# VisionDepth/VisionDepth3D

Hardware: AMD Instinct MI355X
Metric: stereo-pairs/sec end-to-end (depth+warp+fill+mux) (higher is better)
Workload: dtype f32; 1 GPU; 4k-dav2b-dibr; frame=3840x2160, format=Half-SBS, depth_model=depth-anything-v2-base, depth_net_dtype=float32 (the reference's precision), pixel_overlap=True, pixel_streams=2, clip_frames_all_ranks=32, params=render_cli.py defaults + dof_strength 2.0, dense DOF order (parity mode)

## Files before the change

include/vd3d.h:

```cpp
#ifndef VD3D_H
#define VD3D_H

#include <stddef.h>
#include <stdint.h>

#ifdef __cplusplus
extern "C" {
#endif

#define VD3D_ABI_VERSION 6

typedef enum vd3d_status {
  VD3D_OK = 0,
  VD3D_E_INVALID = -1,
  VD3D_E_HIP = -2,
  VD3D_E_NOMEM = -3,
  VD3D_E_UNSUPPORTED = -4
} vd3d_status;

typedef enum vd3d_format {
  VD3D_FMT_HALF_SBS = 0,
  VD3D_FMT_FULL_SBS = 1,
  VD3D_FMT_VR = 2,
  VD3D_FMT_ANAGLYPH = 3,
// ... 93 lines not shown
void vd3d_render_params_default(vd3d_render_params* p);

#define VD3D_STREAM_PRIVATE ((void*)(intptr_t)-1)
int vd3d_ctx_create(int device, void* stream, vd3d_ctx** out);
int vd3d_ctx_destroy(vd3d_ctx* ctx);
int vd3d_sync(vd3d_ctx* ctx);
void* vd3d_ctx_stream(vd3d_ctx* ctx);
int vd3d_ctx_set_stream(vd3d_ctx* ctx, void* stream);
void* vd3d_ctx_pixel_stream(vd3d_ctx* ctx);
void* vd3d_ctx_pixel_stream_k(vd3d_ctx* ctx, int k);

int vd3d_state_reset(vd3d_ctx* ctx);
int vd3d_state_new_clip(vd3d_ctx* ctx);
int vd3d_state_export(vd3d_ctx* ctx, vd3d_state* host_out);
int vd3d_state_import(vd3d_ctx* ctx, const vd3d_state* host_in);
int vd3d_state_planes(vd3d_ctx* ctx, float** tdf_prev, float** norm_prev, int* eye_h, int* eye_w);
int vd3d_last_scalars(vd3d_ctx* ctx, vd3d_frame_scalars* host_out);

int vd3d_pixel_shift(vd3d_ctx* ctx, const float* rgb_chw, const float* depth, int in_h, int in_w,
                     int W, int H, const vd3d_shift_params* p,
                     uint8_t* left_bgr, uint8_t* right_bgr, float* shift_or_null);

int vd3d_render_frame(vd3d_ctx* ctx, const uint8_t* frame_bgr, const void* depth, int depth_fmt,
                      const vd3d_render_params* p, uint8_t* out_bgr);

int vd3d_render_frame_blank(vd3d_ctx* ctx, const uint8_t* frame_bgr, const void* depth, int depth_fmt,
                            const vd3d_render_params* p, uint8_t* out_bgr);

int vd3d_shard_begin(vd3d_ctx* ctx, const vd3d_render_params* p, int n_slots);
int vd3d_shard_pixels(vd3d_ctx* ctx, int slot, const vd3d_render_params* p, uint8_t* out_bgr);
int vd3d_shard_pixels_blank(vd3d_ctx* ctx, int slot, const uint8_t* frame_bgr, const vd3d_render_params* p, uint8_t* out_bgr);
int vd3d_set_pixel_overlap(vd3d_ctx* ctx, int enable);
int vd3d_join_pixels(vd3d_ctx* ctx);
int vd3d_wait_pixels(vd3d_ctx* ctx, int slot);

int vd3d_shard2_p0(vd3d_ctx* ctx, const uint8_t* frame_bgr, const vd3d_render_params* p, int* crop_out_dev);
int vd3d_shard2_set_crops(vd3d_ctx* ctx, const int* crops_all_dev, int n);
int vd3d_shard2_p1(vd3d_ctx* ctx, const uint8_t* frame_bgr, const void* depth, int depth_fmt,
                   const vd3d_render_params* p, int step_idx, int slot, float* q_out_dev);
int vd3d_tdf_plane_export(vd3d_ctx* ctx, float* dst_dev, int eye_h, int eye_w);
int vd3d_tdf_plane_import(vd3d_ctx* ctx, const float* src_dev, int eye_h, int eye_w, int valid);
int vd3d_shard2_r1(vd3d_ctx* ctx, const float* q_all_dev, int n);
int vd3d_shard2_p3(vd3d_ctx* ctx, int slot, int step_idx, const vd3d_render_params* p, long long* m_out_dev);
int vd3d_shard2_p1_batch(vd3d_ctx* ctx, const uint8_t* const* frames_bgr, const void* const* depths, int depth_fmt,
                         const vd3d_render_params* p, int step_idx0, int slot0, int n, float* q_out_dev);
int vd3d_shard2_p3_batch(vd3d_ctx* ctx, int slot0, int step_idx0, int n, const vd3d_render_params* p, long long* m_out_dev);
int vd3d_shard2_r2(vd3d_ctx* ctx, const long long* m_all_dev, const int* own_slot_host, const uint8_t* blank_host_or_null, int n,
                   const vd3d_render_params* p);

int vd3d_heal_missing_pixels(vd3d_ctx* ctx, const float* warped_chw, const float* original_chw, const float* edge_mask_or_null,
                             int H, int W, double heal_strength, float* out_chw);

int vd3d_nv12_to_bgr(vd3d_ctx* ctx, const uint8_t* y_plane, long long y_pitch, const uint8_t* uv_plane, long long uv_pitch, int h, int w,
                     uint8_t* out_bgr);
int vd3d_bgr_to_nv12(vd3d_ctx* ctx, const uint8_t* bgr, int h, int w, uint8_t* y_plane, long long y_pitch, uint8_t* uv_plane,
                     long long uv_pitch);

int vd3d_resize_cubic_u8(vd3d_ctx* ctx, const uint8_t* src, int sh, int sw, int cn, uint8_t* dst, int dh, int dw);
int vd3d_resize_area_u8(vd3d_ctx* ctx, const uint8_t* src_bgr, int sh, int sw, uint8_t* dst_bgr, int dh, int dw);
int vd3d_resize_linear_u8(vd3d_ctx* ctx, const uint8_t* src_bgr, int sh, int sw, uint8_t* dst_bgr, int dh, int dw);
int vd3d_format_3d_output(vd3d_ctx* ctx, const uint8_t* left_bgr, const uint8_t* right_bgr, int h, int w, int format, uint8_t* out_bgr);

int vd3d_esr_preprocess(vd3d_ctx* ctx, int dtype, const uint8_t* frame_bgr, long long pitch_bytes, int h, int w, int channels_last,
                        void* out_rgb);
int vd3d_esr_postprocess(vd3d_ctx* ctx, const float* pred_rgb, int h, int w, int channels_last, int cy, int cx, int ch, int cw,
                         uint8_t* out_bgr, long long pitch_bytes);
int vd3d_add_weighted_u8(vd3d_ctx* ctx, const uint8_t* a, double alpha, const uint8_t* b, double beta, double gamma, long long n,
                         uint8_t* out);
int vd3d_rife_preprocess(vd3d_ctx* ctx, int dtype, const uint8_t* frame1_bgr, const uint8_t* frame2_bgr, int h, int w, int channels_last,
                         void* out6);
int vd3d_rife_postprocess(vd3d_ctx* ctx, const float* pred3, int h, int w, int channels_last, uint8_t* out_bgr);

int vd3d_conv3x3_c64_f16(vd3d_ctx* ctx, const void* x_nhwc, int H, int W, const void* w_frag, const float* bias, const float* slope_or_null,
                         void* y_nhwc);
int vd3d_conv3x3_head_f16(vd3d_ctx* ctx, const void* x_nhwc3, int H, int W, const float* w27x64, const float* bias, const float* slope_or_null,
                          void* y_nhwc64);
int vd3d_esr_tail_f32(vd3d_ctx* ctx, const void* t_nhwc64, const void* x_nhwc3, int H, int W, int r, float* out_planar);
int vd3d_conv3x3_dense_f16(vd3d_ctx* ctx, const void* x, int H, int W, int x_stride, int Cin, const void* w_frag, const float* bias, int Cout,
                           float slope, float alpha, const void* r1_or_null, int r1_stride, float beta, const void* r2_or_null, int r2_stride,
                           int up2, void* y, int y_stride, int y_offset);
int vd3d_nhwc_f16_to_planar3_f32(vd3d_ctx* ctx, const void* t_nhwc32, int H, int W, float* out_planar);

int vd3d_depth_handoff(vd3d_ctx* ctx, const float* pred, int B, int ph, int pw, int H, int W, int invert, uint8_t* out_gray);

int vd3d_tile_gather_cubic_u8(vd3d_ctx* ctx, const uint8_t* frames_bgr, long long pitch_bytes, long long frame_stride_bytes, int B, int H, int W,
                              const int32_t* origins_dev, int n, int ch, int cw, int chs, int cws, uint8_t* out_tiles);
int vd3d_tile_blend_f32(vd3d_ctx* ctx, const float* pred_pool, const int64_t* pred_off_dev, const int32_t* tile_tab_dev, const float* w_pool,
                        int B, int tgt_h, int tgt_w, int tile, int pad, float* out);
int vd3d_depth_normalize_pclip_u8(vd3d_ctx* ctx, const float* planes, int B, int H, int W, float p_lo, float p_hi, int invert, uint8_t* out_gray,
                                  float* lo_hi_dev_or_null);

typedef struct vd3d_letterbox_state {
  int32_t top, bottom;
  int32_t locked_zero, locked_bars;
  int32_t cand_top, cand_bottom, streak;
  int32_t cooldown;
  int32_t have_prev, prev_h, prev_w;
  int32_t reserved;
} vd3d_letterbox_state;
typedef struct vd3d_letterbox_params {
  int32_t min_change, confirm_needed;
  int32_t max_total;
  int32_t cooldown_frames;
} vd3d_letterbox_params;
int vd3d_letterbox_stats(vd3d_ctx* ctx, const uint8_t* frames_bgr, int B, int H, int W, int chain, float* row_mean, float* row_var,
                         uint32_t* row_sat_sum, uint8_t* gray, uint32_t* hist64, uint64_t* mad_sum, float* frame_mean);
int vd3d_canny_u8(vd3d_ctx* ctx, const uint8_t* gray, int B, int H, int W, int low, int high, uint8_t* edges, int32_t* row_counts_or_null);
int vd3d_canny_hysteresis_u8(vd3d_ctx* ctx, const uint8_t* classes, int B, int H, int W, uint8_t* edges, int32_t* row_counts_or_null);
int vd3d_letterbox_track(vd3d_ctx* ctx, const uint8_t* frames_bgr, int B, int H, int W, const vd3d_letterbox_params* params, int32_t* out_bars);
int vd3d_letterbox_state_reset(vd3d_ctx* ctx);
int vd3d_letterbox_state_export(vd3d_ctx* ctx, vd3d_letterbox_state* out, uint32_t* prev_hist64_host_or_null, uint8_t* prev_gray_dev_or_null,
                                long long gray_capacity);
int vd3d_letterbox_state_import(vd3d_ctx* ctx, const vd3d_letterbox_state* in, const uint32_t* prev_hist64_host_or_null,
                                const uint8_t* prev_gray_dev_or_null);
int vd3d_depth_letterbox_fill_u8(vd3d_ctx* ctx, const uint8_t* depth, int B, int H, int W, const int32_t* bars_dev, int bars_stride, uint8_t* out);

typedef enum vd3d_dtype { VD3D_DT_BF16 = 0, VD3D_DT_F32 = 1, VD3D_DT_F16 = 2  } vd3d_dtype;

int vd3d_depth_preprocess(vd3d_ctx* ctx, const uint8_t* frames_bgr, int B, int H, int W, int th, int tw,
                          const float* mean3_host, const float* std3_host, int dtype, void* out_nhwc);

int vd3d_add_layernorm(vd3d_ctx* ctx, int dtype, const void* x, const void* y_or_null, const void* gamma, const void* beta,
                       float eps, int64_t rows, int cols, void* out_sum, void* out_norm);

enum { VD3D_GEMM_EPI_NONE = 0, VD3D_GEMM_EPI_GELU = 1 };
enum { VD3D_X3_BF16X3 = 0, VD3D_X3_FP16X2 = 1 };
int64_t vd3d_gemm_x3_weight_bytes(int N, int K, int mode);
int vd3d_gemm_x3_pack_weights(vd3d_ctx* ctx, const float* W, int N, int K, int mode, void* image);
int vd3d_gemm_x3(vd3d_ctx* ctx, const float* X, int64_t M, int K, const void* w_image, int N, int mode, const float* bias_or_null, int epilogue, float* Y);
int64_t vd3d_attention_x3_workspace_bytes(int B, int T, int H, int D, int mode);
int vd3d_attention_x3(vd3d_ctx* ctx, const float* qkv, int B, int T, int H, int D, float scale, int mode, void* workspace, int64_t workspace_bytes, float* out);
int vd3d_attention_f32(vd3d_ctx* ctx, const float* qkv, int B, int T, int H, int D, float scale, float* out);
int vd3d_attention_f32_form(vd3d_ctx* ctx, const float* qkv, int B, int T, int H, int D, float scale, float* out, int form);

int64_t vd3d_conv3x3_x2_weight_bytes(int Cin, int Cout);
int vd3d_conv3x3_x2_pack_weights(vd3d_ctx* ctx, const float* W, int Cin, int Cout, void* image);
int vd3d_conv3x3_x2(vd3d_ctx* ctx, const float* X, int B, int H, int W, int Cin, const void* w_image, int Cout, float* Y);
int64_t vd3d_conv3x3_x3_weight_bytes(int Cin, int Cout);
int vd3d_conv3x3_x3_pack_weights(vd3d_ctx* ctx, const float* W, int Cin, int Cout, void* image);
int vd3d_conv3x3_x3(vd3d_ctx* ctx, const float* X, int B, int H, int W, int Cin, const void* w_image, int Cout, float* Y);
int64_t vd3d_conv3x3_s2_x3_weight_bytes(int Cin, int Cout);
int vd3d_conv3x3_s2_x3_pack_weights(vd3d_ctx* ctx, const float* W, int Cin, int Cout, void* image);
int vd3d_conv3x3_s2_x3(vd3d_ctx* ctx, const float* X, int B, int H, int W, int Cin, const void* w_image, int Cout, float* Y);

enum { VD3D_IFN_K3S1 = 0, VD3D_IFN_K3S2 = 1, VD3D_IFN_T4S2 = 2 };
int64_t vd3d_conv_ifn_weight_bytes(int kind, int Cin, int Cout);
int vd3d_conv_ifn_pack_weights(vd3d_ctx* ctx, int kind, const float* W, int Cin, int Cout, void* image);
int vd3d_conv_ifn(vd3d_ctx* ctx, int kind, const float* X, int B, int H, int W, int x_stride, int Cin, const void* w_image, const float* bias,
                  const float* slope_or_null, int Cout, const float* r_or_null, int r_stride, float* Y, int y_stride, int y_offset);
int vd3d_rife_warp_pack(vd3d_ctx* ctx, const float* x6, const float* state_or_null, int N, int h, int w, int scale, float* out16);
int vd3d_rife_update(vd3d_ctx* ctx, const float* t, int t_stride, int first, int N, int h, int w, int scale, float* state);
int vd3d_rife_blend(vd3d_ctx* ctx, const float* x6, const float* state, int N, int h, int w, float* out);

int vd3d_upsample_bilinear_nhwc(vd3d_ctx* ctx, int dtype, const void* in, void* out, int B, int ih, int iw, int oh, int ow, int C);

int vd3d_nhwc_bias_act_f32(vd3d_ctx* ctx, const float* y, const float* bias_or_null, const float* r1_or_null, const float* r2_or_null, int relu,
                           int64_t n_pix, int C, float* out, float* relu_out_or_null);
int vd3d_upsample_bilinear_bias_nhwc_f32(vd3d_ctx* ctx, const float* in, const float* bias, float* out, int B, int ih, int iw, int oh, int ow, int C);
int vd3d_dpt_head_tail_f32(vd3d_ctx* ctx, const float* y, const float* b2, const float* w3, float b3, float scale, int64_t n_pix, int C, float* out);

int64_t vd3d_dpt_head_conv_weight_bytes(int Cin, int Cout);
int vd3d_dpt_head_conv_pack_weights(vd3d_ctx* ctx, const float* W, int Cin, int Cout, void* image);
int vd3d_dpt_head_conv_f32(vd3d_ctx* ctx, const float* x, const float* b_in, int B, int ih, int iw, int oh, int ow, int Cin, const void* w_image, int Cout,
                           const float* b2_or_null, const float* w3_or_null, float b3, float scale, float* out);

int vd3d_depth_to_space_bias_nhwc_f32(vd3d_ctx* ctx, const float* y, const float* bias_or_null, int B, int H, int W, int s, int C, float* out);

int vd3d_patchify_f32(vd3d_ctx* ctx, const float* x, int B, int th, int tw, int p, float* rows);

typedef enum vd3d_preview {
  VD3D_PREVIEW_INTERLACED = 0,
  VD3D_PREVIEW_HSBS = 1,
  VD3D_PREVIEW_LR_DIFF = 2,
  VD3D_PREVIEW_FEATHER_BLEND = 3,
  VD3D_PREVIEW_RED_BLUE = 4
} vd3d_preview;
int vd3d_preview_image(vd3d_ctx* ctx, int type, const uint8_t* left_bgr, const uint8_t* right_bgr, int h, int w, uint8_t* out_bgr);
int vd3d_preview_heatmap(vd3d_ctx* ctx, int type, const float* shift_map, int h, int w, const uint8_t* lut_bgr_dev, uint8_t* out_bgr);
int vd3d_preview_arrows(vd3d_ctx* ctx, const uint8_t* left_bgr, const float* shift_map, int h, int w, uint8_t* out_bgr);

int vd3d_finish_frame(vd3d_ctx* ctx, const uint8_t* left_bgr, const uint8_t* right_bgr,
                      const float* depth_norm, int eye_h, int eye_w,
                      const vd3d_render_params* p, double focal_depth, int bar_width, int bar_side,
                      uint8_t* out_bgr);
int vd3d_quantiles(vd3d_ctx* ctx, const float* plane, int64_t n, const float* q_host, int nq, float* out_host);
int vd3d_subject_depth(vd3d_ctx* ctx, const float* plane, int H, int W, float* out_host);
int vd3d_detect_black_bars(vd3d_ctx* ctx, const uint8_t* frame_bgr, int h, int w, int* top_host, int* bottom_host);
int vd3d_stream_copy(vd3d_ctx* ctx, const void* src, void* dst, size_t bytes);
int vd3d_torch_math(vd3d_ctx* ctx, int op, const float* x, float param, float* out, long long n);
int vd3d_torch_math_aten(vd3d_ctx* ctx, int op, const float* x, double param, float* out, long long n, int aten_threads);
int vd3d_set_profiling(vd3d_ctx* ctx, int enable);
int vd3d_debug_tune(int which, int value);
float vd3d_last_stage_ms(vd3d_ctx* ctx, const char* stage);
long vd3d_stage_calls(vd3d_ctx* ctx, const char* stage);
int vd3d_debug_gaussian_kernel1d(int k, float sigma, float* out_host);
int vd3d_debug_exp_torch(const float* x_host, float* out_host, long long n);
int vd3d_debug_planes(vd3d_ctx* ctx, float** D, float** S, uint8_t** L, uint8_t** R, float** rgb_eye, float** dn_cur);

#ifdef __cplusplus
}
#endif
#endif
```

visiondepth3d_amd/_lib.py:

```python
from __future__ import annotations

import ctypes as C
import os

from . import _abi
from ._abi import FrameScalars, LetterboxParams, LetterboxState, RenderParams, ShiftParams, State

_HERE = os.path.dirname(os.path.abspath(__file__))
LIB_PATH = os.environ.get("VD3D_LIB_PATH") or os.path.join(_HERE, "libvd3d_hip.so")

EXPORTS = (
    "vd3d_abi_version", "vd3d_last_error", "vd3d_shift_params_default", "vd3d_render_params_default",
    "vd3d_ctx_create", "vd3d_ctx_destroy", "vd3d_sync", "vd3d_ctx_stream", "vd3d_ctx_set_stream", "vd3d_ctx_pixel_stream", "vd3d_ctx_pixel_stream_k",
    "vd3d_state_reset", "vd3d_state_new_clip", "vd3d_state_export", "vd3d_state_import", "vd3d_state_planes",
    "vd3d_last_scalars", "vd3d_pixel_shift", "vd3d_render_frame", "vd3d_render_frame_blank", "vd3d_depth_handoff", "vd3d_heal_missing_pixels", "vd3d_preview_heatmap", "vd3d_preview_arrows", "vd3d_conv3x3_c64_f16", "vd3d_conv3x3_head_f16", "vd3d_esr_tail_f32", "vd3d_conv3x3_dense_f16", "vd3d_nhwc_f16_to_planar3_f32", "vd3d_nv12_to_bgr", "vd3d_bgr_to_nv12", "vd3d_resize_cubic_u8", "vd3d_resize_area_u8", "vd3d_resize_linear_u8", "vd3d_format_3d_output", "vd3d_esr_preprocess", "vd3d_esr_postprocess", "vd3d_add_weighted_u8", "vd3d_rife_preprocess", "vd3d_rife_postprocess",
    "vd3d_shard_begin", "vd3d_shard_pixels", "vd3d_shard_pixels_blank", "vd3d_tdf_plane_export", "vd3d_tdf_plane_import", "vd3d_set_pixel_overlap", "vd3d_join_pixels", "vd3d_wait_pixels", "vd3d_finish_frame", "vd3d_quantiles",
    "vd3d_subject_depth", "vd3d_shard2_p0", "vd3d_shard2_set_crops", "vd3d_shard2_p1", "vd3d_shard2_p1_batch", "vd3d_shard2_r1", "vd3d_shard2_p3", "vd3d_shard2_p3_batch", "vd3d_shard2_r2", "vd3d_depth_preprocess", "vd3d_tile_gather_cubic_u8", "vd3d_tile_blend_f32", "vd3d_depth_normalize_pclip_u8", "vd3d_letterbox_stats", "vd3d_canny_u8", "vd3d_canny_hysteresis_u8", "vd3d_letterbox_track", "vd3d_letterbox_state_reset", "vd3d_letterbox_state_export", "vd3d_letterbox_state_import", "vd3d_depth_letterbox_fill_u8", "vd3d_add_layernorm", "vd3d_gemm_x3_weight_bytes", "vd3d_gemm_x3_pack_weights", "vd3d_gemm_x3", "vd3d_attention_x3_workspace_bytes", "vd3d_attention_x3", "vd3d_attention_f32", "vd3d_attention_f32_form", "vd3d_conv3x3_x2_weight_bytes", "vd3d_conv3x3_x2_pack_weights", "vd3d_conv3x3_x2", "vd3d_conv3x3_x3_weight_bytes", "vd3d_conv3x3_x3_pack_weights", "vd3d_conv3x3_x3", "vd3d_conv3x3_s2_x3_weight_bytes", "vd3d_conv3x3_s2_x3_pack_weights", "vd3d_conv3x3_s2_x3", "vd3d_conv_ifn_weight_bytes", "vd3d_conv_ifn_pack_weights", "vd3d_conv_ifn", "vd3d_rife_warp_pack", "vd3d_rife_update", "vd3d_rife_blend", "vd3d_upsample_bilinear_nhwc", "vd3d_nhwc_bias_act_f32", "vd3d_upsample_bilinear_bias_nhwc_f32", "vd3d_dpt_head_tail_f32", "vd3d_dpt_head_conv_weight_bytes", "vd3d_dpt_head_conv_pack_weights", "vd3d_dpt_head_conv_f32", "vd3d_depth_to_space_bias_nhwc_f32", "vd3d_patchify_f32", "vd3d_preview_image", "vd3d_detect_black_bars", "vd3d_stream_copy", "vd3d_torch_math", "vd3d_torch_math_aten", "vd3d_debug_gaussian_kernel1d", "vd3d_debug_exp_torch", "vd3d_set_profiling", "vd3d_last_stage_ms", "vd3d_stage_calls",
    "vd3d_debug_planes", "vd3d_debug_tune",
)

_lib = None


class Vd3dError(RuntimeError):
    def __init__(self, code, msg):
        super().__init__(f"libvd3d_hip error {code}: {msg}")
        self.code = code


def lib():
    global _lib
    if _lib is not None:
        return _lib
    if not os.path.exists(LIB_PATH):
        raise ImportError(f"{LIB_PATH} not built: run `python -c 'import __graft_entry__ as g; g.build()'` "
                          "(hipcc --offload-arch=gfx950). There is no CPU fallback.")
    L = C.CDLL(LIB_PATH)
    vp, i32, f32p, u8p = C.c_void_p, C.c_int, C.c_void_p, C.c_void_p
    L.vd3d_abi_version.restype = i32
    L.vd3d_last_error.restype = C.c_char_p
    L.vd3d_ctx_create.argtypes = [i32, vp, C.POINTER(vp)]
    L.vd3d_ctx_destroy.argtypes = [vp]
    L.vd3d_sync.argtypes = [vp]
    L.vd3d_ctx_stream.argtypes = [vp]
    L.vd3d_ctx_stream.restype = vp
    L.vd3d_ctx_set_stream.argtypes = [vp, vp]
    L.vd3d_ctx_pixel_stream.argtypes = [vp]
    L.vd3d_ctx_pixel_stream.restype = vp
    L.vd3d_ctx_pixel_stream_k.argtypes = [vp, i32]
    L.vd3d_ctx_pixel_stream_k.restype = vp
    for n in ("vd3d_state_reset", "vd3d_state_new_clip"):
        getattr(L, n).argtypes = [vp]
    L.vd3d_state_export.argtypes = [vp, C.POINTER(State)]
    L.vd3d_state_import.argtypes = [vp, C.POINTER(State)]
    L.vd3d_state_planes.argtypes = [vp, C.POINTER(vp), C.POINTER(vp), C.POINTER(i32), C.POINTER(i32)]
    L.vd3d_last_scalars.argtypes = [vp, C.POINTER(FrameScalars)]
    L.vd3d_pixel_shift.argtypes = [vp, f32p, f32p, i32, i32, i32, i32, C.POINTER(ShiftParams), u8p, u8p, f32p]
    L.vd3d_render_frame.argtypes = [vp, u8p, vp, i32, C.POINTER(RenderParams), u8p]
    L.vd3d_render_frame_blank.argtypes = [vp, u8p, vp, i32, C.POINTER(RenderParams), u8p]
    L.vd3d_shard_begin.argtypes = [vp, C.POINTER(RenderParams), i32]
    L.vd3d_shard_pixels.argtypes = [vp, i32, C.POINTER(RenderParams), u8p]
    L.vd3d_shard_pixels_blank.argtypes = [vp, i32, u8p, C.POINTER(RenderParams), u8p]
    L.vd3d_tdf_plane_export.argtypes = [vp, f32p, i32, i32]
    L.vd3d_tdf_plane_import.argtypes = [vp, f32p, i32, i32, i32]
    L.vd3d_set_pixel_overlap.argtypes = [vp, i32]
    L.vd3d_join_pixels.argtypes = [vp]
    L.vd3d_wait_pixels.argtypes = [vp, i32]
    L.vd3d_depth_handoff.argtypes = [vp, f32p, i32, i32, i32, i32, i32, i32, u8p]
    L.vd3d_heal_missing_pixels.argtypes = [vp, f32p, f32p, f32p, i32, i32, C.c_double, f32p]
    L.vd3d_resize_cubic_u8.argtypes = [vp, u8p, i32, i32, i32, u8p, i32, i32]
    L.vd3d_nv12_to_bgr.argtypes = [vp, u8p, C.c_longlong, u8p, C.c_longlong, i32, i32, u8p]
    L.vd3d_bgr_to_nv12.argtypes = [vp, u8p, i32, i32, u8p, C.c_longlong, u8p, C.c_longlong]
    L.vd3d_conv3x3_c64_f16.argtypes = [vp, vp, i32, i32, vp, vp, vp, vp]
    L.vd3d_conv3x3_head_f16.argtypes = [vp, vp, i32, i32, vp, vp, vp, vp]
    L.vd3d_esr_tail_f32.argtypes = [vp, vp, vp, i32, i32, i32, vp]
    L.vd3d_conv3x3_dense_f16.argtypes = [vp, vp, i32, i32, i32, i32, vp, vp, i32, C.c_float, C.c_float, vp, i32, C.c_float, vp, i32, i32, vp, i32, i32]
    L.vd3d_nhwc_f16_to_planar3_f32.argtypes = [vp, vp, i32, i32, vp]
    L.vd3d_preview_arrows.argtypes = [vp, u8p, f32p, i32, i32, u8p]
    L.vd3d_preview_heatmap.argtypes = [vp, i32, f32p, i32, i32, u8p, u8p]
    L.vd3d_resize_area_u8.argtypes = [vp, u8p, i32, i32, u8p, i32, i32]
    L.vd3d_resize_linear_u8.argtypes = [vp, u8p, i32, i32, u8p, i32, i32]
    L.vd3d_format_3d_output.argtypes = [vp, u8p, u8p, i32, i32, i32, u8p]
    L.vd3d_esr_preprocess.argtypes = [vp, i32, u8p, C.c_longlong, i32, i32, i32, vp]
    L.vd3d_esr_postprocess.argtypes = [vp, f32p, i32, i32, i32, i32, i32, i32, i32, u8p, C.c_longlong]
    L.vd3d_rife_preprocess.argtypes = [vp, i32, u8p, u8p, i32, i32, i32, vp]
    L.vd3d_rife_postprocess.argtypes = [vp, f32p, i32, i32, i32, u8p]
    L.vd3d_add_weighted_u8.argtypes = [vp, u8p, C.c_double, u8p, C.c_double, C.c_double, C.c_longlong, u8p]
    L.vd3d_finish_frame.argtypes = [vp, u8p, u8p, f32p, i32, i32, C.POINTER(RenderParams), C.c_double, i32, i32, u8p]
    L.vd3d_quantiles.argtypes = [vp, f32p, C.c_int64, C.POINTER(C.c_float), i32, C.POINTER(C.c_float)]
    L.vd3d_subject_depth.argtypes = [vp, f32p, i32, i32, C.POINTER(C.c_float)]
    L.vd3d_shard2_p0.argtypes = [vp, vp, vp, vp]
    L.vd3d_shard2_set_crops.argtypes = [vp, vp, i32]
    L.vd3d_shard2_p1.argtypes = [vp, vp, vp, i32, vp, i32, i32, vp]
    L.vd3d_shard2_p1_batch.argtypes = [vp, vp, vp, i32, vp, i32, i32, i32, vp]
    L.vd3d_shard2_p3_batch.argtypes = [vp, i32, i32, i32, vp, vp]
    L.vd3d_shard2_r1.argtypes = [vp, vp, i32]
    L.vd3d_shard2_p3.argtypes = [vp, i32, i32, vp, vp]
    L.vd3d_shard2_r2.argtypes = [vp, vp, C.POINTER(C.c_int), C.POINTER(C.c_uint8), i32, vp]
    L.vd3d_depth_preprocess.argtypes = [vp, vp, i32, i32, i32, i32, i32, C.POINTER(C.c_float), C.POINTER(C.c_float), i32, vp]
    L.vd3d_tile_gather_cubic_u8.argtypes = [vp, u8p, C.c_longlong, C.c_longlong, i32, i32, i32, vp, i32, i32, i32, i32, i32, u8p]
    L.vd3d_tile_blend_f32.argtypes = [vp, f32p, vp, vp, f32p, i32, i32, i32, i32, i32, f32p]
    L.vd3d_depth_normalize_pclip_u8.argtypes = [vp, f32p, i32, i32, i32, C.c_float, C.c_float, i32, u8p, f32p]
    L.vd3d_letterbox_stats.argtypes = [vp, u8p, i32, i32, i32, i32, f32p, f32p, vp, u8p, vp, vp, f32p]
    L.vd3d_canny_u8.argtypes = [vp, u8p, i32, i32, i32, i32, i32, u8p, vp]
    L.vd3d_canny_hysteresis_u8.argtypes = [vp, u8p, i32, i32, i32, u8p, vp]
    L.vd3d_letterbox_track.argtypes = [vp, u8p, i32, i32, i32, C.POINTER(LetterboxParams), vp]
    L.vd3d_letterbox_state_reset.argtypes = [vp]
    L.vd3d_letterbox_state_export.argtypes = [vp, C.POINTER(LetterboxState), vp, u8p, C.c_longlong]
    L.vd3d_letterbox_state_import.argtypes = [vp, C.POINTER(LetterboxState), vp, u8p]
    L.vd3d_depth_letterbox_fill_u8.argtypes = [vp, u8p, i32, i32, i32, vp, i32, u8p]
    L.vd3d_gemm_x3_weight_bytes.argtypes = [i32, i32, i32]
    L.vd3d_gemm_x3_weight_bytes.restype = C.c_int64
    L.vd3d_gemm_x3_pack_weights.argtypes = [vp, vp, i32, i32, i32, vp]
    L.vd3d_gemm_x3.argtypes = [vp, vp, C.c_int64, i32, vp, i32, i32, vp, i32, vp]
    L.vd3d_attention_x3_workspace_bytes.argtypes = [i32, i32, i32, i32, i32]
    L.vd3d_attention_x3_workspace_bytes.restype = C.c_int64
    L.vd3d_attention_x3.argtypes = [vp, vp, i32, i32, i32, i32, C.c_float, i32, vp, C.c_int64, vp]
    L.vd3d_attention_f32.argtypes = [vp, vp, i32, i32, i32, i32, C.c_float, vp]
    L.vd3d_attention_f32_form.argtypes = [vp, vp, i32, i32, i32, i32, C.c_float, vp, i32]
    L.vd3d_conv3x3_x2_weight_bytes.argtypes = [i32, i32]
    L.vd3d_conv3x3_x2_weight_bytes.restype = C.c_int64
    L.vd3d_conv3x3_x2_pack_weights.argtypes = [vp, vp, i32, i32, vp]
    L.vd3d_conv3x3_x2.argtypes = [vp, vp, i32, i32, i32, i32, vp, i32, vp]
    L.vd3d_conv3x3_x3_weight_bytes.argtypes = [i32, i32]
    L.vd3d_conv3x3_x3_weight_bytes.restype = C.c_int64
    L.vd3d_conv3x3_x3_pack_weights.argtypes = [vp, vp, i32, i32, vp]
    L.vd3d_conv3x3_x3.argtypes = [vp, vp, i32, i32, i32, i32, vp, i32, vp]
    L.vd3d_conv3x3_s2_x3_weight_bytes.argtypes = [i32, i32]
    L.vd3d_conv3x3_s2_x3_weight_bytes.restype = C.c_int64
    L.vd3d_conv3x3_s2_x3_pack_weights.argtypes = [vp, vp, i32, i32, vp]
    L.vd3d_conv3x3_s2_x3.argtypes = [vp, vp, i32, i32, i32, i32, vp, i32, vp]
    L.vd3d_conv_ifn_weight_bytes.argtypes = [i32, i32, i32]
    L.vd3d_conv_ifn_weight_bytes.restype = C.c_int64
    L.vd3d_conv_ifn_pack_weights.argtypes = [vp, i32, vp, i32, i32, vp]
    L.vd3d_conv_ifn.argtypes = [vp, i32, vp, i32, i32, i32, i32, i32, vp, vp, vp, i32, vp, i32, vp, i32, i32]
    L.vd3d_rife_warp_pack.argtypes = [vp, vp, vp, i32, i32, i32, i32, vp]
    L.vd3d_rife_update.argtypes = [vp, vp, i32, i32, i32, i32, i32, i32, vp]
    L.vd3d_rife_blend.argtypes = [vp, vp, vp, i32, i32, i32, vp]
    L.vd3d_add_layernorm.argtypes = [vp, i32, vp, vp, vp, vp, C.c_float, C.c_int64, i32, vp, vp]
    L.vd3d_upsample_bilinear_nhwc.argtypes = [vp, i32, vp, vp, i32, i32, i32, i32, i32, i32]
    L.vd3d_nhwc_bias_act_f32.argtypes = [vp, vp, vp, vp, vp, i32, C.c_int64, i32, vp, vp]
    L.vd3d_upsample_bilinear_bias_nhwc_f32.argtypes = [vp, vp, vp, vp, i32, i32, i32, i32, i32, i32]
    L.vd3d_dpt_head_tail_f32.argtypes = [vp, vp, vp, vp, C.c_float, C.c_float, C.c_int64, i32, vp]
    L.vd3d_dpt_head_conv_weight_bytes.argtypes = [i32, i32]
    L.vd3d_dpt_head_conv_weight_bytes.restype = C.c_int64
    L.vd3d_dpt_head_conv_pack_weights.argtypes = [vp, vp, i32, i32, vp]
    L.vd3d_dpt_head_conv_f32.argtypes = [vp, vp, vp, i32, i32, i32, i32, i32, i32, vp, i32, vp, vp, C.c_float, C.c_float, vp]
    L.vd3d_depth_to_space_bias_nhwc_f32.argtypes = [vp, vp, vp, i32, i32, i32, i32, i32, vp]
    L.vd3d_patchify_f32.argtypes = [vp, vp, i32, i32, i32, i32, vp]
    L.vd3d_preview_image.argtypes = [vp, i32, vp, vp, i32, i32, vp]
    L.vd3d_detect_black_bars.argtypes = [vp, vp, i32, i32, C.POINTER(C.c_int), C.POINTER(C.c_int)]
    L.vd3d_stream_copy.argtypes = [vp, vp, vp, C.c_size_t]
    L.vd3d_torch_math.argtypes = [vp, i32, vp, C.c_float, vp, C.c_longlong]
    L.vd3d_torch_math_aten.argtypes = [vp, i32, vp, C.c_double, vp, C.c_longlong, i32]
    L.vd3d_debug_gaussian_kernel1d.argtypes = [i32, C.c_float, vp]
    L.vd3d_debug_exp_torch.argtypes = [vp, vp, C.c_longlong]
    L.vd3d_debug_tune.argtypes = [i32, i32]
    L.vd3d_set_profiling.argtypes = [vp, i32]
    L.vd3d_last_stage_ms.argtypes = [vp, C.c_char_p]
    L.vd3d_last_stage_ms.restype = C.c_float
    L.vd3d_stage_calls.argtypes = [vp, C.c_char_p]
    L.vd3d_stage_calls.restype = C.c_long
    L.vd3d_debug_planes.argtypes = [vp] + [C.POINTER(vp)] * 6
    L.vd3d_shift_params_default.argtypes = [C.POINTER(ShiftParams)]
    L.vd3d_render_params_default.argtypes = [C.POINTER(RenderParams)]
    if L.vd3d_abi_version() != _abi.ABI_VERSION:
        raise ImportError("libvd3d_hip.so ABI version mismatch")
    if os.environ.get("VD3D_TUNE"):
        if L.vd3d_debug_tune(-1, 0) != 0:
            raise ImportError("VD3D_TUNE is set but this libvd3d_hip.so was built without -DVD3D_DEV_KNOBS (bash tools/build_ab.sh dev -DVD3D_DEV_KNOBS; VD3D_LIB_PATH=...)")
        for kv in filter(None, os.environ["VD3D_TUNE"].split(",")):
            k, v = kv.split(":")
            if L.vd3d_debug_tune(int(k), int(v)) != 0:
                raise ImportError(f"VD3D_TUNE: unknown knob {k}")
    _lib = L
    return L


def check(rc):
    if rc != 0:
        raise Vd3dError(rc, lib().vd3d_last_error().decode(errors="replace"))
```

visiondepth3d_amd/csrc/vd3d_api.hip:

```cpp
#include <hip/hip_runtime.h>

#include <cmath>
#include <cstdarg>
#include <cstddef>
#include <cstdio>
#include <cstring>
#include <cstdlib>
#include <map>
#include <string>
#include <vector>

#include "vd3d_kernels.h"

#define VD3D_EXPORT extern "C" __attribute__((visibility("default")))

static thread_local char g_err[512] = "";
static int set_err(int code, const char* fmt, ...) {
  va_list ap;
  va_start(ap, fmt);
  vsnprintf(g_err, sizeof g_err, fmt, ap);
  va_end(ap);
  return code;
}
#define HIPCHK(x)                                                                                     \
// ... 1188 lines not shown
VD3D_EXPORT int vd3d_resize_linear_u8(vd3d_ctx* c, const uint8_t* src_bgr, int sh, int sw, uint8_t* dst_bgr, int dh, int dw) {
  if (!c || !src_bgr || !dst_bgr || sh < 1 || sw < 1 || dh < 1 || dw < 1 || src_bgr == dst_bgr) return set_err(VD3D_E_INVALID, "bad argument");
  if ((long long)sh * sw * 3 >= (1ll << 31) || (long long)dh * dw * 3 >= (1ll << 31)) return set_err(VD3D_E_INVALID, "image too large");
  HIPCHK(hipSetDevice(c->device));
  vd_launch_resize_linear_u8(c->stream, src_bgr, sh, sw, dst_bgr, dh, dw);
  HIPCHK(hipGetLastError());
  return 0;
}

VD3D_EXPORT int vd3d_format_3d_output(vd3d_ctx* c, const uint8_t* left_bgr, const uint8_t* right_bgr, int h, int w, int format, uint8_t* out_bgr) {
  if (!c || !left_bgr || !right_bgr || !out_bgr || h < 1 || w < 1) return set_err(VD3D_E_INVALID, "bad argument");
  if (format < 0 || format > VD3D_FMT_INTERLACED) return set_err(VD3D_E_INVALID, "unknown format %d", format);
  HIPCHK(hipSetDevice(c->device));
  int rc = join_pixels(c);
  if (rc) return rc;
  const uint8_t *L = left_bgr, *R = right_bgr;
  int eh = h, ew = w;
  if (format == VD3D_FMT_VR && (h != 1600 || w != 1440)) {
    const size_t ne = (size_t)1600 * 1440 * 3;
    if (c->fmt_cap < 2 * ne) { HIPCHK(re_alloc(&c->fmt_eyes, 2 * ne)); c->fmt_cap = 2 * ne; }
    vd_launch_resize_linear_u8(c->stream, left_bgr, h, w, c->fmt_eyes, 1600, 1440);
    vd_launch_resize_linear_u8(c->stream, right_bgr, h, w, c->fmt_eyes + ne, 1600, 1440);
    L = c->fmt_eyes; R = c->fmt_eyes + ne; eh = 1600; ew = 1440;
  }
  vd3d_render_params p;
  vd3d_render_params_default(&p);
  p.format = format; p.warp_w = ew; p.warp_h = eh; p.fit_w = ew; p.fit_h = eh;
  p.out_w = (format == VD3D_FMT_HALF_SBS || format == VD3D_FMT_FULL_SBS || format == VD3D_FMT_VR) ? 2 * ew : ew; p.out_h = eh;
  vd_finish_consts fc;
  memset(&fc, 0, sizeof fc);
  fc.sharp_kn = 0.f; fc.sharp_kc = 1.f;
  vd_launch_sharp_mux(c->stream, L, R, p, fc, out_bgr, 0, true);
  HIPCHK(hipGetLastError());
  return 0;
}

VD3D_EXPORT int vd3d_esr_preprocess(vd3d_ctx* c, int dtype, const uint8_t* frame_bgr, long long pitch_bytes, int h, int w, int channels_last,
                                    void* out_rgb) {
  if (!c || !frame_bgr || !out_rgb || h < 1 || w < 1 || pitch_bytes < 3ll * w) return set_err(VD3D_E_INVALID, "bad argument");
  HIPCHK(hipSetDevice(c->device));
  StageTimer t(c, "esr_pre");
  if (!vd_launch_esr_pre(c->stream, dtype, frame_bgr, pitch_bytes, h, w, channels_last ? 1 : 0, out_rgb)) return set_err(VD3D_E_INVALID, "bad dtype %d", dtype);
  HIPCHK(hipGetLastError());
  return 0;
}

VD3D_EXPORT int vd3d_esr_postprocess(vd3d_ctx* c, const float* pred_rgb, int h, int w, int channels_last, int cy, int cx, int ch, int cw,
                                     uint8_t* out_bgr, long long pitch_bytes) {
  if (!c || !pred_rgb || !out_bgr || h < 1 || w < 1 || cy < 0 || cx < 0 || ch < 1 || cw < 1 || cy + ch > h || cx + cw > w || pitch_bytes < 3ll * cw)
    return set_err(VD3D_E_INVALID, "bad argument");
  HIPCHK(hipSetDevice(c->device));
  StageTimer t(c, "esr_post");
  vd_launch_esr_post(c->stream, pred_rgb, h, w, channels_last ? 1 : 0, cy, cx, ch, cw, out_bgr, pitch_bytes);
  HIPCHK(hipGetLastError());
  return 0;
}

VD3D_EXPORT int vd3d_rife_preprocess(vd3d_ctx* c, int dtype, const uint8_t* frame1_bgr, const uint8_t* frame2_bgr, int h, int w, int channels_last,
                                     void* out6) {
  if (!c || !frame1_bgr || !frame2_bgr || !out6 || h < 1 || w < 1) return set_err(VD3D_E_INVALID, "bad argument");
  HIPCHK(hipSetDevice(c->device));
  if (!vd_launch_rife_pre(c->stream, dtype, frame1_bgr, frame2_bgr, h, w, channels_last ? 1 : 0, out6)) return set_err(VD3D_E_INVALID, "bad dtype %d", dtype);
  HIPCHK(hipGetLastError());
  return 0;
}
VD3D_EXPORT int vd3d_rife_postprocess(vd3d_ctx* c, const float* pred3, int h, int w, int channels_last, uint8_t* out_bgr) {
  if (!c || !pred3 || !out_bgr || h < 1 || w < 1) return set_err(VD3D_E_INVALID, "bad argument");
  HIPCHK(hipSetDevice(c->device));
  vd_launch_rife_post(c->stream, pred3, h, w, channels_last ? 1 : 0, out_bgr);
  HIPCHK(hipGetLastError());
  return 0;
}

VD3D_EXPORT int vd3d_add_weighted_u8(vd3d_ctx* c, const uint8_t* a, double alpha, const uint8_t* b, double beta, double gamma, long long n,
                                     uint8_t* out) {
  if (!c || !a || !b || !out || n < 1) return set_err(VD3D_E_INVALID, "bad argument");
  HIPCHK(hipSetDevice(c->device));
  StageTimer t(c, "add_weighted");
  vd_launch_add_weighted_u8(c->stream, a, (float)alpha, b, (float)beta, (float)gamma, n, out);
  HIPCHK(hipGetLastError());
  return 0;
}

VD3D_EXPORT int vd3d_depth_handoff(vd3d_ctx* c, const float* pred, int B, int ph, int pw, int H, int W, int invert, uint8_t* out_gray) {
  if (!c || !pred || !out_gray || B < 1 || ph < 1 || pw < 1 || H < 1 || W < 1) return set_err(VD3D_E_INVALID, "bad argument");
  HIPCHK(hipSetDevice(c->device));
  if (B > c->mm_cap) { HIPCHK(re_alloc(&c->mm, (size_t)3 * B)); c->mm_cap = B; }
  StageTimer t(c, "handoff");
  vd_launch_depth_handoff(c->stream, pred, B, ph, pw, H, W, invert ? 1 : 0, c->mm, out_gray);
  HIPCHK(hipGetLastError());
  return 0;
}

VD3D_EXPORT int vd3d_tile_gather_cubic_u8(vd3d_ctx* c, const uint8_t* frames_bgr, long long pitch_bytes, long long frame_stride_bytes, int B, int H, int W,
                                          const int32_t* origins_dev, int n, int ch, int cw, int chs, int cws, uint8_t* out_tiles) {
  if (!c || !frames_bgr || !origins_dev || !out_tiles || B < 1 || H < 1 || W < 1 || n < 1 || ch < 1 || cw < 1 || chs < 1 || cws < 1)
    return set_err(VD3D_E_INVALID, "bad argument");
  if (ch > H || cw > W || pitch_bytes < 3ll * W || (B > 1 && frame_stride_bytes < pitch_bytes * H))
    return set_err(VD3D_E_INVALID, "tile_gather: crop %dx%d of a %dx%d frame, pitch %lld, frame stride %lld", cw, ch, W, H, pitch_bytes, frame_stride_bytes);
  if ((long long)n * chs * cws * 3 >= (1ll << 31)) return set_err(VD3D_E_INVALID, "tile batch too large");
  HIPCHK(hipSetDevice(c->device));
  StageTimer t(c, "tile_gather");
  if (!vd_launch_tile_gather(c->stream, frames_bgr, pitch_bytes, frame_stride_bytes, B, H, W, origins_dev, n, ch, cw, chs, cws, out_tiles))
    return set_err(VD3D_E_UNSUPPORTED, "tile_gather: %d tiles in one launch (<= 65535)", n);
  HIPCHK(hipGetLastError());
  return 0;
}

VD3D_EXPORT int vd3d_tile_blend_f32(vd3d_ctx* c, const float* pred_pool, const int64_t* pred_off_dev, const int32_t* tile_tab_dev, const float* w_pool,
                                    int B, int tgt_h, int tgt_w, int tile, int pad, float* out) {
  if (!c || !pred_pool || !pred_off_dev || !tile_tab_dev || !w_pool || !out || B < 1 || B > 65535 || tgt_h < 1 || tgt_w < 1 || tile < 1 || pad < 0)
    return set_err(VD3D_E_INVALID, "bad argument");
  if ((reinterpret_cast<uintptr_t>(tile_tab_dev) & 15) != 0) return set_err(VD3D_E_INVALID, "tile_blend: the tile table must be 16-byte aligned");
  if ((long long)tgt_h * tgt_w >= (1ll << 31)) return set_err(VD3D_E_INVALID, "plane too large");
  const int core = tile - 2 * pad > 1 ? tile - 2 * pad : 1;
  if ((tile + core - 1) / core > 4)
    return set_err(VD3D_E_UNSUPPORTED, "tile_blend: tile %d with pad %d puts %d tiles over a pixel per axis (built for <= 4: pad <= 3/8 tile)", tile, pad,
                   (tile + core - 1) / core);
  HIPCHK(hipSetDevice(c->device));
  StageTimer t(c, "tile_blend");
  vd_launch_tile_blend(c->stream, pred_pool, reinterpret_cast<const long long*>(pred_off_dev), tile_tab_dev, w_pool, B, tgt_h, tgt_w, tile, core, out);
  HIPCHK(hipGetLastError());
  return 0;
}

VD3D_EXPORT int vd3d_depth_normalize_pclip_u8(vd3d_ctx* c, const float* planes, int B, int H, int W, float p_lo, float p_hi, int invert, uint8_t* out_gray,
                                              float* lo_hi_dev_or_null) {
  if (!c || !planes || !out_gray || B < 1 || B > 65535 || H < 1 || W < 1 || !(p_lo >= 0.f && p_lo <= p_hi && p_hi <= 100.f))
    return set_err(VD3D_E_INVALID, "bad argument");
  const long long n = (long long)H * W;
  if (n >= (1ll << 31)) return set_err(VD3D_E_INVALID, "plane too large");
  HIPCHK(hipSetDevice(c->device));
  if (B > c->pclip_cap) { HIPCHK(re_alloc(&c->pclip_ws, (size_t)B * VD_PCLIP_WS_WORDS)); c->pclip_cap = B; }
  uint32_t rank[VD_PCLIP_NR];
  float g[2];
  const float pc[2] = {p_lo, p_hi};
  const float last = (float)(n - 1);
  for (int k = 0; k < 2; ++k) {
    const float q = pc[k] / 100.0f;
    const float vi = last * q;
    uint32_t k0, k1;
    if (vi >= last) { k0 = k1 = (uint32_t)(n - 1); g[k] = 0.f; }
    else { const float fl = floorf(vi); k0 = (uint32_t)fl; k1 = k0 + 1; g[k] = vi - fl; }
    if (k1 > (uint32_t)(n - 1)) k1 = (uint32_t)(n - 1);
    rank[1 + 2 * k] = k0; rank[2 + 2 * k] = k1;
  }
  rank[0] = 0; rank[5] = (uint32_t)(n - 1);
  StageTimer t(c, "pclip_u8");
  vd_launch_pclip_u8(c->stream, planes, B, n, rank, g[0], g[1], invert ? 1 : 0, c->pclip_ws, out_gray, lo_hi_dev_or_null);
  HIPCHK(hipGetLastError());
  return 0;
}

static int lb_check(vd3d_ctx* c, const void* p0, const void* p1, int B, int H, int W) {
  if (!c || !p0 || !p1 || B < 1 || H < 1 || W < 1) return set_err(VD3D_E_INVALID, "bad argument");
  if (!vd_lb_size_ok(B, H, W)) return set_err(VD3D_E_UNSUPPORTED, "letterbox: %d frames of %dx%d (built for W <= 8192, H <= 8192, B <= 4096)", B, W, H);
  return 0;
}

VD3D_EXPORT int vd3d_letterbox_stats(vd3d_ctx* c, const uint8_t* frames_bgr, int B, int H, int W, int chain, float* row_mean, float* row_var,
                                     uint32_t* row_sat_sum, uint8_t* gray, uint32_t* hist64, uint64_t* mad_sum, float* frame_mean) {
  if (!row_mean || !row_var || !row_sat_sum || !hist64 || !mad_sum || !frame_mean) return set_err(VD3D_E_INVALID, "bad argument");
  if (int rc = lb_check(c, frames_bgr, gray, B, H, W)) return rc;
  HIPCHK(hipSetDevice(c->device));
  StageTimer t(c, "letterbox_stats");
  HIPCHK(vd_lb_stats(&c->lb, c->stream, frames_bgr, B, H, W, chain ? 1 : 0, row_mean, row_var, row_sat_sum, gray, hist64,
                     reinterpret_cast<unsigned long long*>(mad_sum), frame_mean));
  if (chain) HIPCHK(vd_lb_stats_commit(&c->lb, c->stream, gray, hist64, B, H, W));
  return 0;
}

VD3D_EXPORT int vd3d_canny_u8(vd3d_ctx* c, const uint8_t* gray, int B, int H, int W, int low, int high, uint8_t* edges, int32_t* row_counts_or_null) {
  if (int rc = lb_check(c, gray, edges, B, H, W)) return rc;
  if (low < 0 || high < low || high > 1442) return set_err(VD3D_E_INVALID, "canny: thresholds %d, %d (0 <= low <= high <= 1442)", low, high);
  HIPCHK(hipSetDevice(c->device));
  StageTimer t(c, "canny");
  HIPCHK(vd_lb_canny(&c->lb, c->stream, gray, B, H, W, low, high, edges, row_counts_or_null));
  return 0;
}

VD3D_EXPORT int vd3d_canny_hysteresis_u8(vd3d_ctx* c, const uint8_t* classes, int B, int H, int W, uint8_t* edges, int32_t* row_counts_or_null) {
  if (int rc = lb_check(c, classes, edges, B, H, W)) return rc;
  if (classes == edges) return set_err(VD3D_E_INVALID, "canny_hysteresis: the edge map needs its own buffer");
  HIPCHK(hipSetDevice(c->device));
  StageTimer t(c, "canny_hysteresis");
  HIPCHK(vd_lb_hysteresis(&c->lb, c->stream, classes, B, H, W, edges, row_counts_or_null));
  return 0;
}

VD3D_EXPORT int vd3d_letterbox_track(vd3d_ctx* c, const uint8_t* frames_bgr, int B, int H, int W, const vd3d_letterbox_params* params, int32_t* out_bars) {
  if (!params) return set_err(VD3D_E_INVALID, "bad argument");
  if (int rc = lb_check(c, frames_bgr, out_bars, B, H, W)) return rc;
  HIPCHK(hipSetDevice(c->device));
  StageTimer t(c, "letterbox_track");
  HIPCHK(vd_lb_track(&c->lb, c->stream, frames_bgr, B, H, W, params, out_bars));
  return 0;
}

VD3D_EXPORT int vd3d_letterbox_state_reset(vd3d_ctx* c) {
  if (!c) return set_err(VD3D_E_INVALID, "NULL context");
  HIPCHK(hipSetDevice(c->device));
  HIPCHK(vd_lb_state_reset(&c->lb, c->stream));
  return 0;
}

VD3D_EXPORT int vd3d_letterbox_state_export(vd3d_ctx* c, vd3d_letterbox_state* out, uint32_t* prev_hist64_host_or_null, uint8_t* prev_gray_dev_or_null,
                                            long long gray_capacity) {
  if (!c || !out) return set_err(VD3D_E_INVALID, "bad argument");
  HIPCHK(hipSetDevice(c->device));
  HIPCHK(vd_lb_state_export(&c->lb, c->stream, out, prev_hist64_host_or_null, prev_gray_dev_or_null, gray_capacity));
  return 0;
}

VD3D_EXPORT int vd3d_letterbox_state_import(vd3d_ctx* c, const vd3d_letterbox_state* in, const uint32_t* prev_hist64_host_or_null,
                                            const uint8_t* prev_gray_dev_or_null) {
  if (!c || !in) return set_err(VD3D_E_INVALID, "bad argument");
  if (in->have_prev && prev_gray_dev_or_null && !vd_lb_size_ok(1, in->prev_h, in->prev_w)) return set_err(VD3D_E_INVALID, "letterbox state: previous frame %dx%d", in->prev_w, in->prev_h);
  HIPCHK(hipSetDevice(c->device));
  HIPCHK(vd_lb_state_import(&c->lb, c->stream, in, prev_hist64_host_or_null, prev_gray_dev_or_null));
  return 0;
}

VD3D_EXPORT int vd3d_depth_letterbox_fill_u8(vd3d_ctx* c, const uint8_t* depth, int B, int H, int W, const int32_t* bars_dev, int bars_stride, uint8_t* out) {
  if (!bars_dev || bars_stride < 0 || bars_stride == 1) return set_err(VD3D_E_INVALID, "bad argument");
  if (int rc = lb_check(c, depth, out, B, H, W)) return rc;
  if (depth == out) return set_err(VD3D_E_INVALID, "depth_letterbox_fill: the output needs its own buffer");
  HIPCHK(hipSetDevice(c->device));
  StageTimer t(c, "letterbox_fill");
  HIPCHK(vd_lb_fill(&c->lb, c->stream, depth, B, H, W, bars_dev, bars_stride, out));
  return 0;
}

VD3D_EXPORT int vd3d_depth_preprocess(vd3d_ctx* c, const uint8_t* frames_bgr, int B, int H, int W, int th, int tw,
                                      const float* mean3_host, const float* std3_host, int dtype, void* out_nhwc) {
  if (dtype != VD3D_DT_BF16 && dtype != VD3D_DT_F32) return set_err(VD3D_E_INVALID, "bad dtype %d", dtype);
  if (!c || !frames_bgr || !mean3_host || !std3_host || !out_nhwc || B < 1 || H < 1 || W < 1 || th < 1 || tw < 1)
    return set_err(VD3D_E_INVALID, "bad argument");
  HIPCHK(hipSetDevice(c->device));
  StageTimer t(c, "depth_prep");
  if (!vd_launch_depth_prep(c->stream, frames_bgr, B, H, W, th, tw, mean3_host, std3_host, dtype, out_nhwc))
    return set_err(VD3D_E_UNSUPPORTED, "depth_preprocess: %dx%d -> %dx%d exceeds the antialias tap budget", W, H, tw, th);
  HIPCHK(hipGetLastError());
  return 0;
}

VD3D_EXPORT int vd3d_add_layernorm(vd3d_ctx* c, int dtype, const void* x, const void* y_or_null, const void* gamma, const void* beta,
                                   float eps, int64_t rows, int cols, void* out_sum, void* out_norm) {
  if (dtype != VD3D_DT_BF16 && dtype != VD3D_DT_F32) return set_err(VD3D_E_INVALID, "bad dtype %d", dtype);
  if (!c || !x || !gamma || !beta || !out_norm || rows < 1 || (y_or_null && !out_sum)) return set_err(VD3D_E_INVALID, "bad argument");
  if (!vd_launch_add_layernorm(c->stream, dtype, x, y_or_null, gamma, beta, eps, (long long)rows, cols, out_sum, out_norm))
    return set_err(VD3D_E_UNSUPPORTED, "add_layernorm: cols %d not in {384,768,1024}", cols);
  HIPCHK(hipGetLastError());
  return 0;
}

VD3D_EXPORT int64_t vd3d_conv3x3_x2_weight_bytes(int Cin, int Cout) { return (int64_t)vd_conv3x3_x2_weight_bytes(Cin, Cout); }

VD3D_EXPORT int vd3d_conv3x3_x2_pack_weights(vd3d_ctx* c, const float* W, int Cin, int Cout, void* image) {
  if (!c || !W || !image) return set_err(VD3D_E_INVALID, "bad argument");
  HIPCHK(hipSetDevice(c->device));
  if (!vd_launch_conv3x3_x2_pack(c->stream, W, Cin, Cout, image))
    return set_err(VD3D_E_UNSUPPORTED, "conv3x3_x2: C_in %d must be a positive multiple of 16 and C_out %d one of 64, 128", Cin, Cout);
  HIPCHK(hipGetLastError());
  return 0;
}

VD3D_EXPORT int vd3d_conv3x3_x2(vd3d_ctx* c, const float* X, int B, int H, int W, int Cin, const void* w_image, int Cout, float* Y) {
  if (!c || !X || !w_image || !Y) return set_err(VD3D_E_INVALID, "bad argument");
  HIPCHK(hipSetDevice(c->device));
  if (!vd_launch_conv3x3_x2(c->stream, X, B, H, W, Cin, w_image, Cout, Y))
    return set_err(VD3D_E_UNSUPPORTED, "conv3x3_x2: C_in %d (multiple of 16), C_out %d (64 | 128), B %d <= 65535, 16-byte aligned input and image", Cin, Cout, B);
  HIPCHK(hipGetLastError());
  return 0;
}

VD3D_EXPORT int64_t vd3d_conv3x3_x3_weight_bytes(int Cin, int Cout) { return (int64_t)vd_conv3x3_x3_weight_bytes(Cin, Cout); }

static int conv3x3_x3_shape_err(int Cin, int Cout) {
  return set_err(VD3D_E_UNSUPPORTED, "conv3x3_x3: shape not built: C_in %d must be a positive multiple of 16 and C_out %d one of 32, 64, 128, 256", Cin, Cout);
}

VD3D_EXPORT int vd3d_conv3x3_x3_pack_weights(vd3d_ctx* c, const float* W, int Cin, int Cout, void* image) {
  if (!c || !W || !image) return set_err(VD3D_E_INVALID, "bad argument");
  if (vd_conv3x3_x3_weight_bytes(Cin, Cout) < 0) return conv3x3_x3_shape_err(Cin, Cout);
  if (reinterpret_cast<uintptr_t>(image) & 15) return set_err(VD3D_E_UNSUPPORTED, "conv3x3_x3: the weight image must be 16-byte aligned");
  HIPCHK(hipSetDevice(c->device));
  if (!vd_launch_conv3x3_x3_pack(c->stream, W, Cin, Cout, image)) return set_err(VD3D_E_HIP, "conv3x3_x3: the weight pack launch failed");
  HIPCHK(hipGetLastError());
  return 0;
}

VD3D_EXPORT int vd3d_conv3x3_x3(vd3d_ctx* c, const float* X, int B, int H, int W, int Cin, const void* w_image, int Cout, float* Y) {
  if (!c || !X || !w_image || !Y) return set_err(VD3D_E_INVALID, "bad argument");
  if (vd_conv3x3_x3_weight_bytes(Cin, Cout) < 0) return conv3x3_x3_shape_err(Cin, Cout);
  if (B < 1 || B > 65535) return set_err(VD3D_E_UNSUPPORTED, "conv3x3_x3: batch %d must be 1 .. 65535 (one grid row per frame)", B);
  if (H < 1 || W < 1) return set_err(VD3D_E_UNSUPPORTED, "conv3x3_x3: map %d x %d must be at least 1 x 1", H, W);
  if ((reinterpret_cast<uintptr_t>(X) & 15) || (reinterpret_cast<uintptr_t>(w_image) & 15) || (reinterpret_cast<uintptr_t>(Y) & 3))
    return set_err(VD3D_E_UNSUPPORTED, "conv3x3_x3: the input and the weight image must be 16-byte aligned (the output 4-byte)");
  HIPCHK(hipSetDevice(c->device));
  if (!vd_launch_conv3x3_x3(c->stream, X, B, H, W, Cin, w_image, Cout, Y)) return set_err(VD3D_E_HIP, "conv3x3_x3: the dynamic LDS opt-in or the launch failed");
  HIPCHK(hipGetLastError());
  return 0;
}

VD3D_EXPORT int64_t vd3d_conv3x3_s2_x3_weight_bytes(int Cin, int Cout) { return (int64_t)vd_conv3x3_s2_x3_weight_bytes(Cin, Cout); }

static int conv3x3_s2_x3_shape_err(int Cin, int Cout) {
  return set_err(VD3D_E_UNSUPPORTED, "conv3x3_s2_x3: shape not built: C_in %d must be a positive multiple of 16 (at most 65536) and C_out %d a positive multiple of 128 (at most 1024)",
                 Cin, Cout);
}

VD3D_EXPORT int vd3d_conv3x3_s2_x3_pack_weights(vd3d_ctx* c, const float* W, int Cin, int Cout, void* image) {
  if (!c || !W || !image) return set_err(VD3D_E_INVALID, "bad argument");
  if (vd_conv3x3_s2_x3_weight_bytes(Cin, Cout) < 0) return conv3x3_s2_x3_shape_err(Cin, Cout);
  if (reinterpret_cast<uintptr_t>(image) & 15) return set_err(VD3D_E_UNSUPPORTED, "conv3x3_s2_x3: the weight image must be 16-byte aligned");
  HIPCHK(hipSetDevice(c->device));
  if (!vd_launch_conv3x3_s2_x3_pack(c->stream, W, Cin, Cout, image)) return set_err(VD3D_E_HIP, "conv3x3_s2_x3: the weight pack launch failed");
  HIPCHK(hipGetLastError());
  return 0;
}

VD3D_EXPORT int vd3d_conv3x3_s2_x3(vd3d_ctx* c, const float* X, int B, int H, int W, int Cin, const void* w_image, int Cout, float* Y) {
  if (!c || !X || !w_image || !Y) return set_err(VD3D_E_INVALID, "bad argument");
  if (vd_conv3x3_s2_x3_weight_bytes(Cin, Cout) < 0) return conv3x3_s2_x3_shape_err(Cin, Cout);
  if (B < 1 || B > 65535) return set_err(VD3D_E_UNSUPPORTED, "conv3x3_s2_x3: batch %d must be 1 .. 65535 (one grid row per frame)", B);
  if (H < 1 || W < 1) return set_err(VD3D_E_UNSUPPORTED, "conv3x3_s2_x3: map %d x %d must be at least 1 x 1", H, W);
// ... 444 lines not shown
```

visiondepth3d_amd/csrc/vd3d_depthprep.hip:

```cpp
#include "vd3d_dev.h"
#include "vd3d_kernels.h"

#define DP_TX 32
#define DP_TY 8
#define DP_KMAX 24

struct vd_prep_args {
  int B, H, W, th, tw;
  float scale_h, scale_w;
  float mean[3], stdv[3];
  int in_rows_max, in_cols_max;
};

VD_DEV float dp_cubic(float x) {
  const float a = -0.5f;
  x = fabsf(x);
  if (x < 1.f) return ((a + 2.f) * x - (a + 3.f)) * x * x + 1.f;
  if (x < 2.f) return (((x - 5.f) * x + 8.f) * x - 4.f) * a;
  return 0.f;
}
VD_DEV int dp_weights(int i, int in, float scale, float* w, int* first) {
  const float support = scale >= 1.f ? 2.f * scale : 2.f;
  const float invscale = scale >= 1.f ? 1.f / scale : 1.f;
  const float center = scale * ((float)i + 0.5f);
  int xmin = (int)(center - support + 0.5f); xmin = xmin < 0 ? 0 : xmin;
  int xend = (int)(center + support + 0.5f); xend = xend > in ? in : xend;
  int n = xend - xmin; n = n > DP_KMAX ? DP_KMAX : n;
  float total = 0.f;
  for (int j = 0; j < n; ++j) { const float v = dp_cubic(((float)(j + xmin) - center + 0.5f) * invscale); w[j] = v; total += v; }
  for (int j = 0; j < n; ++j) w[j] = total != 0.f ? w[j] / total : w[j];
  *first = xmin;
  return n;
}
VD_DEV uint16_t dp_bf16(float f) {
  const uint32_t b = __float_as_uint(f);
  return (uint16_t)((b + 0x7fffu + ((b >> 16) & 1u)) >> 16);
}

VD_DEV void dp_store(uint16_t* o, float f) { *o = dp_bf16(f); }
VD_DEV void dp_store(float* o, float f) { *o = f; }

template <typename OT>
__global__ __launch_bounds__(256) void k_depth_prep(const uint8_t* __restrict__ frames, vd_prep_args a, OT* __restrict__ out) {
  extern __shared__ unsigned char smem[];
  float* wx = reinterpret_cast<float*>(smem);
  float* wy = wx + DP_TX * DP_KMAX;
  int* x0s = reinterpret_cast<int*>(wy + DP_TY * DP_KMAX);
  int* y0s = x0s + 2 * DP_TX;
  float* hb = reinterpret_cast<float*>(y0s + 2 * DP_TY);
  uint8_t* tile = reinterpret_cast<uint8_t*>(hb + (size_t)a.in_rows_max * DP_TX * 3);
  const int tid = threadIdx.x;
  const int ox0 = blockIdx.x * DP_TX, oy0 = blockIdx.y * DP_TY, b = blockIdx.z;
  if (tid < DP_TX) {
    int f = 0, n = 0;
    if (ox0 + tid < a.tw) n = dp_weights(ox0 + tid, a.W, a.scale_w, wx + tid * DP_KMAX, &f);
    x0s[tid] = f; x0s[DP_TX + tid] = n;
  } else if (tid >= 64 && tid < 64 + DP_TY) {
    const int t = tid - 64;
    int f = 0, n = 0;
    if (oy0 + t < a.th) n = dp_weights(oy0 + t, a.H, a.scale_h, wy + t * DP_KMAX, &f);
    y0s[t] = f; y0s[DP_TY + t] = n;
  }
  __syncthreads();
  const int nx = min(DP_TX, a.tw - ox0), ny = min(DP_TY, a.th - oy0);
  const int c_lo = x0s[0], c_hi = x0s[nx - 1] + x0s[DP_TX + nx - 1];
  const int r_lo = y0s[0], r_hi = y0s[ny - 1] + y0s[DP_TY + ny - 1];
  const int ncol = min(c_hi - c_lo, a.in_cols_max), nrow = min(r_hi - r_lo, a.in_rows_max);
  const uint8_t* src = frames + (size_t)b * a.H * a.W * 3;
  const int rowbytes = ncol * 3;
  for (int t = tid; t < nrow * rowbytes; t += 256) {
    const int r = t / rowbytes, cb = t - r * rowbytes;
    tile[(size_t)r * a.in_cols_max * 3 + cb] = src[((size_t)(r_lo + r) * a.W + c_lo) * 3 + cb];
  }
  __syncthreads();
  for (int t = tid; t < nrow * DP_TX; t += 256) {
    const int r = t / DP_TX, ox = t - r * DP_TX;
    float s0 = 0.f, s1 = 0.f, s2 = 0.f;
    if (ox < nx) {
      const int n = x0s[DP_TX + ox];
      const uint8_t* p = tile + (size_t)r * a.in_cols_max * 3 + (size_t)(x0s[ox] - c_lo) * 3;
      const float* w = wx + ox * DP_KMAX;
      for (int j = 0; j < n; ++j) {
        const float wj = w[j];
        s0 += (float)p[3 * j + 2] * wj; s1 += (float)p[3 * j + 1] * wj; s2 += (float)p[3 * j] * wj;
      }
    }
    float* h = hb + ((size_t)r * DP_TX + ox) * 3;
    h[0] = s0; h[1] = s1; h[2] = s2;
  }
  __syncthreads();
  const int ox = tid & (DP_TX - 1), oy = tid / DP_TX;
  if (ox < nx && oy < ny) {
    const int n = y0s[DP_TY + oy], rb = y0s[oy] - r_lo;
    const float* w = wy + oy * DP_KMAX;
    float s[3] = {0.f, 0.f, 0.f};
    for (int j = 0; j < n; ++j) {
      const float* h = hb + ((size_t)(rb + j) * DP_TX + ox) * 3;
      const float wj = w[j];
      s[0] += h[0] * wj; s[1] += h[1] * wj; s[2] += h[2] * wj;
    }
    OT* o = out + (((size_t)b * a.th + (oy0 + oy)) * a.tw + (ox0 + ox)) * 3;
#pragma unroll
    for (int c = 0; c < 3; ++c) dp_store(o + c, ((s[c] / 255.0f) - a.mean[c]) / a.stdv[c]);
  }
}

bool vd_launch_depth_prep(hipStream_t s, const uint8_t* frames, int B, int H, int W, int th, int tw, const float mean[3],
                          const float stdv[3], int dtype, void* out_nhwc) {
  if (dtype != VD3D_DT_BF16 && dtype != VD3D_DT_F32) return false;
  vd_prep_args a;
  a.B = B; a.H = H; a.W = W; a.th = th; a.tw = tw;
  a.scale_h = (float)H / (float)th; a.scale_w = (float)W / (float)tw;
  const float sup_w = a.scale_w >= 1.f ? 2.f * a.scale_w : 2.f, sup_h = a.scale_h >= 1.f ? 2.f * a.scale_h : 2.f;
  if ((int)(2.f * sup_w) + 2 > DP_KMAX || (int)(2.f * sup_h) + 2 > DP_KMAX) return false;
  for (int c = 0; c < 3; ++c) { a.mean[c] = mean[c]; a.stdv[c] = stdv[c]; }
  a.in_cols_max = (int)(a.scale_w * DP_TX + 2.f * sup_w) + 4;
  a.in_rows_max = (int)(a.scale_h * DP_TY + 2.f * sup_h) + 4;
  size_t lds = sizeof(float) * (DP_TX + DP_TY) * DP_KMAX + sizeof(int) * 2 * (DP_TX + DP_TY) +
               sizeof(float) * (size_t)a.in_rows_max * DP_TX * 3 + (size_t)a.in_rows_max * a.in_cols_max * 3;
  lds = (lds + 15) & ~(size_t)15;
  if (lds > 150 * 1024) return false;
  static bool attr[64] = {false};
  int dev = 0;
  (void)hipGetDevice(&dev);
  if (dev >= 0 && dev < 64 && !attr[dev]) {
    (void)hipFuncSetAttribute((const void*)k_depth_prep<uint16_t>, hipFuncAttributeMaxDynamicSharedMemorySize, 160 * 1024);
    (void)hipFuncSetAttribute((const void*)k_depth_prep<float>, hipFuncAttributeMaxDynamicSharedMemorySize, 160 * 1024);
    attr[dev] = true;
  }
  dim3 g((tw + DP_TX - 1) / DP_TX, (th + DP_TY - 1) / DP_TY, B);
  if (dtype == VD3D_DT_F32) hipLaunchKernelGGL(k_depth_prep<float>, g, dim3(256), lds, s, frames, a, reinterpret_cast<float*>(out_nhwc));
  else hipLaunchKernelGGL(k_depth_prep<uint16_t>, g, dim3(256), lds, s, frames, a, reinterpret_cast<uint16_t*>(out_nhwc));
  return true;
}
```

visiondepth3d_amd/csrc/vd3d_handoff.hip:

```cpp
#include "vd3d_dev.h"
#include "vd3d_kernels.h"
#include "vd3d_cubic.h"

struct vd_handoff_args { int B, ph, pw, H, W, invert, same; float sh, sw; };

VD_DEV uint32_t f2key(float v) { uint32_t b = __float_as_uint(v); return (b & 0x80000000u) ? ~b : (b | 0x80000000u); }
VD_DEV float key2f(uint32_t k) { uint32_t b = (k & 0x80000000u) ? (k & 0x7fffffffu) : ~k; return __uint_as_float(b); }

__global__ void k_handoff_init(uint32_t* mm, int B) {
  int i = blockIdx.x * blockDim.x + threadIdx.x;
  if (i < B) { mm[3 * i] = 0xffffffffu; mm[3 * i + 1] = 0u; mm[3 * i + 2] = 0u; }
}

#define HO_ROWS 32
template <bool WRITE>
__global__ __launch_bounds__(256) void k_handoff(const float* __restrict__ pred, vd_handoff_args a, uint32_t* __restrict__ mm,
                                                 uint8_t* __restrict__ out) {
  const int b = blockIdx.z;
  const float* p = pred + (size_t)b * a.ph * a.pw;
  const int xq = (blockIdx.x * 64 + (threadIdx.x & 63)) * 4;
  float bmn = INFINITY, bmx = -INFINITY;
  int bbad = 0;
  for (int ry_ = 0; ry_ < HO_ROWS / 4; ++ry_) {
  const int y = blockIdx.y * HO_ROWS + ry_ * 4 + (threadIdx.x >> 6);
  float v[4] = {0.f, 0.f, 0.f, 0.f};
  const bool row_ok = y < a.H;
  if (row_ok && xq < a.W) {
    if (a.same) {
#pragma unroll
      for (int q = 0; q < 4; ++q) if (xq + q < a.W) v[q] = p[(size_t)y * a.W + xq + q];
    } else {
      const float ry = vd_fma(a.sh, (float)y + 0.5f, -0.5f);
      const float fy = floorf(ry);
      float cy[4];
      cubic_coeffs(ry - fy, cy);
#pragma unroll
      for (int q = 0; q < 4; ++q) if (xq + q < a.W) v[q] = bicubic_at(p, a.ph, a.pw, a.sw, cy, (int)fy, xq + q);
    }
  }
  if (!WRITE) {
    float mn = INFINITY, mx = -INFINITY;
    int bad = 0;
    if (row_ok)
#pragma unroll
      for (int q = 0; q < 4; ++q)
        if (xq + q < a.W) { bad |= (v[q] != v[q]); mn = v[q] < mn ? v[q] : mn; mx = v[q] > mx ? v[q] : mx; }
    bmn = fminf(bmn, mn); bmx = fmaxf(bmx, mx); bbad |= bad;
  } else {
    if (!row_ok || xq >= a.W) continue;
    const float mn = key2f(mm[3 * b]), mx = key2f(mm[3 * b + 1]);
    const bool flat = mm[3 * b + 2] != 0u || (mx - mn) < (float)1e-6;
    const float den = (mx - mn) + (float)1e-6;
    uint32_t pack = 0;
#pragma unroll
    for (int q = 0; q < 4; ++q) {
      uint8_t u = 0;
      if (!flat) {
        float n = ((v[q] - mn) / den) * 255.f;
        n = n < 0.f ? 0.f : (n > 255.f ? 255.f : n);
        u = (uint8_t)n;
      }
      if (a.invert) u = (uint8_t)(255 - u);
      pack |= (uint32_t)u << (8 * q);
    }
    uint8_t* o = out + (size_t)b * a.H * a.W + (size_t)y * a.W + xq;
    if (xq + 3 < a.W && (((size_t)b * a.H * a.W + (size_t)y * a.W + xq) & 3) == 0) *reinterpret_cast<uint32_t*>(o) = pack;
    else for (int q = 0; q < 4 && xq + q < a.W; ++q) o[q] = (uint8_t)(pack >> (8 * q));
  }
  }
  if (!WRITE) {
    __shared__ float smn[4], smx[4];
    __shared__ int sbad[4];
    for (int off = 32; off > 0; off >>= 1) {
      bmn = fminf(bmn, __shfl_down(bmn, off, 64));
      bmx = fmaxf(bmx, __shfl_down(bmx, off, 64));
      bbad |= __shfl_down(bbad, off, 64);
    }
    if ((threadIdx.x & 63) == 0) { smn[threadIdx.x >> 6] = bmn; smx[threadIdx.x >> 6] = bmx; sbad[threadIdx.x >> 6] = bbad; }
    __syncthreads();
    if (threadIdx.x == 0) {
      const float mn = fminf(fminf(smn[0], smn[1]), fminf(smn[2], smn[3]));
      const float mx = fmaxf(fmaxf(smx[0], smx[1]), fmaxf(smx[2], smx[3]));
      if (mn <= mx) { atomicMin(&mm[3 * b], f2key(mn)); atomicMax(&mm[3 * b + 1], f2key(mx)); }
      if (sbad[0] | sbad[1] | sbad[2] | sbad[3]) atomicOr(&mm[3 * b + 2], 1u);
    }
  }
}

void vd_launch_depth_handoff(hipStream_t s, const float* pred, int B, int ph, int pw, int H, int W, int invert, uint32_t* mm,
                             uint8_t* out) {
  vd_handoff_args a;
  a.B = B; a.ph = ph; a.pw = pw; a.H = H; a.W = W; a.invert = invert; a.same = (ph == H && pw == W);
  a.sh = (float)ph / (float)H; a.sw = (float)pw / (float)W;
  hipLaunchKernelGGL(k_handoff_init, dim3((B + 63) / 64), dim3(64), 0, s, mm, B);
  dim3 g((W + 255) / 256, (H + HO_ROWS - 1) / HO_ROWS, B);
  hipLaunchKernelGGL(k_handoff<false>, g, dim3(256), 0, s, pred, a, mm, out);
  hipLaunchKernelGGL(k_handoff<true>, g, dim3(256), 0, s, pred, a, mm, out);
}
```

visiondepth3d_amd/csrc/vd3d_kernels.h:

```cpp
#pragma once
#include <hip/hip_runtime.h>

#include <initializer_list>
#include <mutex>

#include "vd3d_work.h"

struct vd_lds_fn { const void* fn; int bytes; };
inline bool vd_lds_optin(std::initializer_list<vd_lds_fn> fns, bool (&done)[64]) {
  static std::mutex mu;
  int dev = 0;
  if (hipGetDevice(&dev) != hipSuccess || dev < 0 || dev >= 64) return false;
  std::lock_guard<std::mutex> lock(mu);
  if (!done[dev]) {
    for (const vd_lds_fn& f : fns)
      if (hipFuncSetAttribute(f.fn, hipFuncAttributeMaxDynamicSharedMemorySize, f.bytes) != hipSuccess) return false;
    done[dev] = true;
  }
  return true;
}

enum { VD_ST_A0 = 0, VD_ST_B0, VD_ST_A1, VD_ST_B1, VD_ST_A2, VD_ST_B2,
       VD_ST_AQ, VD_ST_BQ, VD_ST_BS };
#define PL_KMAX_HOST 129
// ... 83 lines not shown
    for (int c = 0; c < 3; ++c) {
      const int sc = 2 - c;
      float p00 = vd_u8_unit((float)frame[i00 * 3 + sc]), p01 = vd_u8_unit((float)frame[i01 * 3 + sc]);
      float p10 = vd_u8_unit((float)frame[i10 * 3 + sc]), p11 = vd_u8_unit((float)frame[i11 * 3 + sc]);
      rgb_eye[c * ne + o] = vd_bilerp_sel(pm_c, p00, p01, p10, p11, tx.w0, tx.w1, ty.w0, ty.w1);
    }
  }
  const float cur = vd_bilerp_sel(pm_d, vd_depth_at(depth, fmt, i00), vd_depth_at(depth, fmt, i01), vd_depth_at(depth, fmt, i10),
                                  vd_depth_at(depth, fmt, i11), tx.w0, tx.w1, ty.w0, ty.w1);
  const float prev = tdf_valid ? tdf_prev[o] : cur;
  const float nv = 0.5f * prev + (float)(1 - 0.5) * cur;
  tdf[o] = nv;
  return nv;
}
#endif

void vd_launch_shard2_r1(hipStream_t s, vd_dev_work* w, const float* q_all, int n, float* etab);
void vd_launch_shard2_r2(hipStream_t s, vd_dev_work* w, const long long* m_all, const float* etab, const int* own_slot_host,
                         const uint8_t* blank_host_or_null, int n, vd_dev_work* slot_work, const vd_stage_args& a);
void vd_launch_autocrop(hipStream_t s, const uint8_t* frame, int h, int wd, double target_ratio, uint32_t* rowflag, vd_dev_work* w,
                        int* crop_out = nullptr);
void vd_set_batch_grid_div(int v);
void vd_launch_chain_eye(hipStream_t s, const vd_batch& b, int fmt, const vd3d_render_params& p, const vd_stage_args& a);
void vd_launch_chain_work(hipStream_t s, const vd_batch& b, int have_eye, int ih, int iw, int H, int W, float mid, float gamma,
                          const vd_stage_args& a);

void vd_launch_hist_eye_d(hipStream_t s, bool passB, const float* tdf, long long n, vd_dev_work* w, uint32_t* histA, uint32_t* histB);
void vd_launch_hist_work_s1(hipStream_t s, bool passB, const float* D, int H, int W, vd_dev_work* w, uint32_t* histA, uint32_t* histB);
void vd_launch_scalar_stage(hipStream_t s, vd_dev_work* w, const uint32_t* histA, const uint32_t* histB, const vd_stage_args& a);

struct vd_finish_consts {
  int nlev;
  int ksz[4];
  float kern[4][32];
  float w2[4][81];
  float fw, imax;
  float sat, con, bri;
  float sharp_kn, sharp_kc;
};
struct vd_shift_consts {
  float mid, fg, mg, bg, fgm, bgm, pb, half_width, fs, ma, mb;
  int edge;
};
vd_shift_consts vd_shift_consts_of(const vd3d_shift_params& p, int W);
void vd_launch_shift(hipStream_t s, const float* D, int H, int W, const vd_dev_work* w, const vd3d_shift_params& p, float* S);
struct vd_shift_fold { const vd_dev_work* work; vd3d_shift_params sp; float* S_out; };
bool vd_warp_fold_ok(int ih, int iw, int H, int W, const vd3d_shift_params& warp_p, const vd3d_shift_params& shift_p);
void vd_launch_e2(hipStream_t s, const float* D, const float* S, int H, int W, float fs, float* e2L, float* e2R);
void vd_launch_pool(hipStream_t s, const float* e2L, const float* e2R, int H, int W, int k, float* bL, float* bR);
void vd_launch_warp(hipStream_t s, const float* rgb, int ih, int iw, const float* S, const float* bL, const float* bR, int H, int W,
                    int feather, uint8_t* L, uint8_t* R);
bool vd_launch_warp_fused(hipStream_t s, const float* rgb, int ih, int iw, const float* D, const float* S, int H, int W,
                          const vd3d_shift_params& p, uint8_t* L, uint8_t* R, const float* E2 = nullptr, const vd_shift_fold* fold = nullptr);
bool vd_warp_fused_ok(int ih, int iw, int H, int W, const vd3d_shift_params& p);
void vd_launch_e2w(hipStream_t s, const float* D, const float* S, int H, int W, float feather_strength, float* E2);
void vd_set_warp_pre_th(int th);
void vd_set_warp_order(int v);
void vd_set_warp_nofeather_th(int th);
#ifdef __cplusplus
#include <vector>
bool vd_aten_plan_build(int eh, int ew, int T, std::vector<int>& pieces_flat, int* n_small, int* n_big, int* nr_crop, int* nr_mad);
#endif
void vd_launch_aten_sums(hipStream_t s, const vd_batch& b, const vd_stage_args& a);
void vd_set_finish_persist(int k);
void vd_set_finish_xcd(int on);
void vd_set_conv_mode(int v);
void vd_launch_dof_grade(hipStream_t s, const uint8_t* eye_in, const float* dn, int eh, int ew, int H, int W,
                         const vd_finish_consts& fc, const vd_dev_work* w, float focal_override, int use_override,
                         int bar_width, int bar_side, uint8_t* eye_out, int dense = 0, const float* dense_wtab = nullptr);
void vd_launch_dof_grade_dense(hipStream_t s, const uint8_t* L_in, const uint8_t* R_in, const float* dn, int eh, int ew, int H, int W,
                               const vd_finish_consts& fc, const vd_dev_work* w, float focal_override, int use_override,
                               int bar_width, int bar_side, uint8_t* L_out, uint8_t* R_out, const float* wtab);
#define VD_D4_WTAB_FLOATS (4 * 31 * 32)
bool vd_launch_sharp_fit(hipStream_t s, const uint8_t* gL, const uint8_t* gR, const vd3d_render_params& p, const vd_finish_consts& fc, uint8_t* out);
void vd_launch_sharp_mux(hipStream_t s, const uint8_t* gL, const uint8_t* gR, const vd3d_render_params& p,
                         const vd_finish_consts& fc, uint8_t* out, int presharp_pitch = 0, bool identity_fit = false);
void vd_launch_stream_copy(hipStream_t s, const void* src, void* dst, size_t bytes);
void vd_launch_interp_planes(hipStream_t s, const float* src, int C, int ih, int iw, float* dst, int oh, int ow, int premult);
void vd_launch_torch_math_aten(hipStream_t s, int op, const float* x, double p, float* out, long long n, int threads);
void vd_launch_torch_math(hipStream_t s, int op, const float* x, float p, float* out, long long n);
void vd_launch_blank_eye(hipStream_t s, const uint8_t* src, int h, int w, const vd_dev_work* wk, uint8_t* dst);

bool vd_launch_preview(hipStream_t s, int type, const uint8_t* L, const uint8_t* R, int h, int w, uint8_t* out);
bool vd_launch_depth_prep(hipStream_t s, const uint8_t* frames, int B, int H, int W, int th, int tw, const float mean[3],
                          const float stdv[3], int dtype, void* out_nhwc);
long long vd_gemm_x3_weight_bytes(int N, int K, int mode);
bool vd_launch_gemm_x3_pack_w(hipStream_t s, const float* W, int N, int K, void* img, int mode);
bool vd_launch_gemm_x3(hipStream_t s, const float* X, long long M, int K, const void* wimg, int N, const float* bias, int epilogue, float* Y, int mode);
long long vd_conv3x3_x2_weight_bytes(int Cin, int Cout);
bool vd_launch_conv3x3_x2_pack(hipStream_t s, const float* W, int Cin, int Cout, void* img);
bool vd_launch_conv3x3_x2(hipStream_t s, const float* X, int B, int H, int W, int Cin, const void* wimg, int Cout, float* Y);
long long vd_conv3x3_x3_weight_bytes(int Cin, int Cout);
bool vd_launch_conv3x3_x3_pack(hipStream_t s, const float* W, int Cin, int Cout, void* img);
bool vd_launch_conv3x3_x3(hipStream_t s, const float* X, int B, int H, int W, int Cin, const void* wimg, int Cout, float* Y);
long long vd_conv3x3_s2_x3_weight_bytes(int Cin, int Cout);
bool vd_launch_conv3x3_s2_x3_pack(hipStream_t s, const float* W, int Cin, int Cout, void* img);
bool vd_launch_conv3x3_s2_x3(hipStream_t s, const float* X, int B, int H, int W, int Cin, const void* wimg, int Cout, float* Y);
long long vd_dpt_head_conv_weight_bytes(int Cin, int Cout);
bool vd_launch_dpt_head_conv_pack(hipStream_t s, const float* W, int Cin, int Cout, void* img);
bool vd_dpt_head_conv_shape_ok(int B, int ih, int iw, int oh, int ow, int Cin, int Cout, bool tail);
bool vd_launch_dpt_head_conv_f32(hipStream_t s, const float* x, const float* b_in, int B, int ih, int iw, int oh, int ow, int Cin, const void* wimg, int Cout,
                                 const float* b2, const float* w3, float b3, float scale, float* out);
long long vd_conv_ifn_weight_bytes(int kind, int Cin, int Cout);
bool vd_launch_conv_ifn_pack(hipStream_t s, int kind, const float* W, int Cin, int Cout, void* img);
bool vd_launch_conv_ifn(hipStream_t s, int kind, const float* X, int B, int H, int W, int x_stride, int Cin, const void* wimg, const float* bias,
                        const float* slope, int Cout, const float* R, int r_stride, float* Y, int y_stride, int y_offset);
void vd_launch_rife_warp_pack(hipStream_t s, const float* X, const float* S, int first, int N, int h, int w, int Hp, int Wp, int scale, float* out);
void vd_launch_rife_update(hipStream_t s, const float* T, int t_stride, int first, int N, int Hp, int Wp, int scale, float* S);
void vd_launch_rife_blend(hipStream_t s, const float* X, const float* S, int N, int h, int w, int Hp, int Wp, float* out);
long long vd_attn_x3_workspace_bytes(int B, int T, int H, int D, int mode);
bool vd_launch_attn_x3(hipStream_t s, const float* qkv, int B, int T, int H, int D, float scale, void* ws, float* out, int mode);
bool vd_launch_attn_f32(hipStream_t s, const float* qkv, int B, int T, int H, int D, float scale, float* out, int form);
bool vd_launch_add_layernorm(hipStream_t s, int dtype, const void* x, const void* y, const void* gamma, const void* beta, float eps,
                             long long rows, int cols, void* out_sum, void* out_norm);
bool vd_launch_upsample_bilinear_nhwc(hipStream_t s, int dtype, const void* in, void* out, int B, int ih, int iw, int oh, int ow, int C);
bool vd_launch_bias_act_f32(hipStream_t s, const float* y, const float* bias, const float* r1, const float* r2, int relu, long long n_pix, int C,
                            float* out, float* relu_out);
bool vd_launch_upsample_bilinear_bias_nhwc_f32(hipStream_t s, const float* in, const float* bias, float* out, int B, int ih, int iw, int oh, int ow, int C);
bool vd_launch_head_tail_f32(hipStream_t s, const float* y, const float* b2, const float* w3, float b3, float scale, long long n_pix, int C, float* out);
bool vd_launch_depth_to_space_bias_f32(hipStream_t s, const float* y, const float* bias, int B, int H, int W, int f, int C, float* out);
bool vd_launch_patchify_f32(hipStream_t s, const float* x, int B, int th, int tw, int p, float* out);
void vd_launch_depth_handoff(hipStream_t s, const float* pred, int B, int ph, int pw, int H, int W, int invert, uint32_t* mm,
                             uint8_t* out);

#define VD_PCLIP_NR 6
#define VD_PCLIP_WS_WORDS (4 * VD_PCLIP_NR * 256)
bool vd_launch_tile_gather(hipStream_t s, const uint8_t* frames, long long pitch, long long fstride, int B, int H, int W, const int32_t* origins,
                           int n, int ch, int cw, int chs, int cws, uint8_t* out);
void vd_launch_tile_blend(hipStream_t s, const float* pool, const long long* pred_off, const int32_t* tab, const float* wpool, int B, int H, int W,
                          int tile, int core, float* out);
void vd_launch_pclip_u8(hipStream_t s, const float* planes, int B, long long n, const uint32_t rank[VD_PCLIP_NR], float g_lo, float g_hi, int invert,
                        uint32_t* ws, uint8_t* out, float* lohi);

struct vd_lb_ws;
void vd_lb_free(vd_lb_ws* w);
bool vd_lb_size_ok(int B, int H, int W);
hipError_t vd_lb_state_reset(vd_lb_ws** ws, hipStream_t s);
hipError_t vd_lb_state_export(vd_lb_ws** ws, hipStream_t s, vd3d_letterbox_state* out, uint32_t* prev_hist64, uint8_t* prev_gray_dev, long long gray_cap);
hipError_t vd_lb_state_import(vd_lb_ws** ws, hipStream_t s, const vd3d_letterbox_state* in, const uint32_t* prev_hist64, const uint8_t* prev_gray_dev);
hipError_t vd_lb_stats(vd_lb_ws** ws, hipStream_t s, const uint8_t* frames, int B, int H, int W, int chain, float* row_mean, float* row_var,
                       uint32_t* row_sat, uint8_t* gray, uint32_t* hist, unsigned long long* mad, float* fmean);
hipError_t vd_lb_stats_commit(vd_lb_ws** ws, hipStream_t s, const uint8_t* gray, const uint32_t* hist, int B, int H, int W);
hipError_t vd_lb_canny(vd_lb_ws** ws, hipStream_t s, const uint8_t* gray, int B, int H, int W, int low, int high, uint8_t* edges, int32_t* rowcnt);
hipError_t vd_lb_hysteresis(vd_lb_ws** ws, hipStream_t s, const uint8_t* cls, int B, int H, int W, uint8_t* edges, int32_t* rowcnt);
hipError_t vd_lb_track(vd_lb_ws** ws, hipStream_t s, const uint8_t* frames, int B, int H, int W, const vd3d_letterbox_params* p, int32_t* out_bars);
hipError_t vd_lb_fill(vd_lb_ws** ws, hipStream_t s, const uint8_t* depth, int B, int H, int W, const int32_t* bars_dev, int bars_stride, uint8_t* out);

bool vd_launch_finish_fused(hipStream_t s, const uint8_t* L, const uint8_t* R, const float* dn, int eh, int ew,
                            const vd3d_render_params& p, const vd_finish_consts& fc, const vd_dev_work* w, float focal,
                            int use_override, int bar_w, int bar_s, uint8_t* out, int dense, const float* w2_dev);

bool vd_launch_conv3x3_c64_f16(hipStream_t s, const void* x, int H, int W, const void* wfrag, const float* bias, const float* slope_or_null, void* y);
void vd_launch_conv3x3_head_f16(hipStream_t s, const void* x, int H, int W, const float* w27, const float* bias, const float* slope_or_null, void* y);
void vd_launch_esr_tail_f32(hipStream_t s, const void* t, const void* x, int H, int W, int r, float* out);
bool vd_launch_conv3x3_dense_f16(hipStream_t s, const void* x, int H, int W, int x_stride, int Cin, const void* wfrag, const float* bias, int Cout,
                                 float slope, float alpha, const void* r1, int r1_stride, float beta, const void* r2, int r2_stride, int up2,
                                 void* y, int y_stride, int y_offset);
void vd_launch_nhwc_f16_to_planar3_f32(hipStream_t s, const void* t, int H, int W, float* out);
void vd_launch_nv12_to_bgr(hipStream_t s, const uint8_t* y, const uint8_t* uv, int h, int w, long long y_pitch, long long uv_pitch, uint8_t* out);
void vd_launch_bgr_to_nv12(hipStream_t s, const uint8_t* bgr, int h, int w, uint8_t* y, uint8_t* uv, long long y_pitch, long long uv_pitch);
bool vd_launch_preview_heatmap(hipStream_t s, int type, const float* shift, int h, int w, const uint8_t* lut_dev, uint32_t* mm, uint8_t* out);
void vd_launch_preview_arrows(hipStream_t s, const uint8_t* left, const float* shift, int h, int w, uint8_t* out);
bool vd_launch_resize_cubic_u8(hipStream_t s, const uint8_t* src, int sh, int sw, int cn, uint8_t* dst, int dh, int dw);
bool vd_launch_resize_area_u8(hipStream_t s, const uint8_t* src, int sh, int sw, uint8_t* dst, int dh, int dw);
void vd_launch_resize_linear_u8(hipStream_t s, const uint8_t* src, int sh, int sw, uint8_t* dst, int dh, int dw);
bool vd_launch_rife_pre(hipStream_t s, int dtype, const uint8_t* f1, const uint8_t* f2, int h, int w, int hwc, void* out);
void vd_launch_rife_post(hipStream_t s, const float* pred, int h, int w, int hwc, uint8_t* dst);
bool vd_launch_esr_pre(hipStream_t s, int dtype, const uint8_t* src, long long pitch, int h, int w, int hwc, void* out);
void vd_launch_esr_post(hipStream_t s, const float* pred, int h, int w, int hwc, int cy, int cx, int ch, int cw, uint8_t* dst, long long pitch);
void vd_launch_add_weighted_u8(hipStream_t s, const uint8_t* a, float alpha, const uint8_t* b, float beta, float gamma, long long n, uint8_t* out);

void vd_launch_heal(hipStream_t s, const float* warped, const float* orig, const float* edge_or_null, int H, int W, float hs, float* out);
```

visiondepth3d_amd/csrc/vd3d_netops.hip:

```cpp
#include "vd3d_dev.h"
#include "vd3d_kernels.h"

VD_DEV float bf2f(uint32_t h) { return __uint_as_float(h << 16); }
VD_DEV uint32_t f2bf(float f) { const uint32_t b = __float_as_uint(f); return (b + 0x7fffu + ((b >> 16) & 1u)) >> 16; }
VD_DEV float wave_sum_f(float v) {
  for (int off = 32; off > 0; off >>= 1) v += __shfl_xor(v, off, 64);
  return v;
}

template <int NJ>
__global__ __launch_bounds__(256) void k_add_layernorm(const uint32_t* __restrict__ x, const uint32_t* __restrict__ y,
                                                       const uint32_t* __restrict__ gamma, const uint32_t* __restrict__ beta,
                                                       float eps, long long rows, uint32_t* __restrict__ out_sum,
                                                       uint32_t* __restrict__ out_norm) {
  const int lane = threadIdx.x & 63;
  const long long row = (long long)blockIdx.x * 4 + (threadIdx.x >> 6);
  if (row >= rows) return;
  const size_t base = (size_t)row * (NJ * 64);
  float v[2 * NJ];
  float sum = 0.f;
#pragma unroll
  for (int j = 0; j < NJ; ++j) {
    const uint32_t a = x[base + lane + 64 * j];
    float lo = bf2f(a & 0xffffu), hi = bf2f(a >> 16);
// ... 29 lines not shown
  const int lane = threadIdx.x & 63;
  const long long row = (long long)blockIdx.x * 4 + (threadIdx.x >> 6);
  if (row >= rows) return;
  const size_t base = (size_t)row * (NJ * 64);
  float v[2 * NJ];
  float sum = 0.f;
#pragma unroll
  for (int j = 0; j < NJ; ++j) {
    float2 a = x[base + lane + 64 * j];
    if (y) {
      const float2 b = y[base + lane + 64 * j];
      a.x += b.x; a.y += b.y;
      out_sum[base + lane + 64 * j] = a;
    }
    v[2 * j] = a.x; v[2 * j + 1] = a.y;
    sum += a.x + a.y;
  }
  const float n = (float)(NJ * 128);
  const float mean = wave_sum_f(sum) / n;
  float sq = 0.f;
#pragma unroll
  for (int j = 0; j < 2 * NJ; ++j) { const float d = v[j] - mean; sq += d * d; }
  const float rstd = 1.0f / sqrtf(wave_sum_f(sq) / n + eps);
#pragma unroll
  for (int j = 0; j < NJ; ++j) {
    const float2 g = gamma[lane + 64 * j], b = beta[lane + 64 * j];
    out_norm[base + lane + 64 * j] = make_float2((v[2 * j] - mean) * rstd * g.x + b.x, (v[2 * j + 1] - mean) * rstd * g.y + b.y);
  }
}

bool vd_launch_add_layernorm(hipStream_t s, int dtype, const void* x, const void* y, const void* gamma, const void* beta, float eps,
                             long long rows, int cols, void* out_sum, void* out_norm) {
  const dim3 g((unsigned)((rows + 3) / 4)), b(256);
  if (dtype == VD3D_DT_F32) {
    const float2 *xx = (const float2*)x, *yy = (const float2*)y, *gg = (const float2*)gamma, *bb = (const float2*)beta;
    float2 *os = (float2*)out_sum, *on = (float2*)out_norm;
    switch (cols) {
      case 384: hipLaunchKernelGGL(k_add_layernorm_f32<3>, g, b, 0, s, xx, yy, gg, bb, eps, rows, os, on); return true;
      case 768: hipLaunchKernelGGL(k_add_layernorm_f32<6>, g, b, 0, s, xx, yy, gg, bb, eps, rows, os, on); return true;
      case 1024: hipLaunchKernelGGL(k_add_layernorm_f32<8>, g, b, 0, s, xx, yy, gg, bb, eps, rows, os, on); return true;
      default: return false;
    }
  }
  if (dtype != VD3D_DT_BF16) return false;
  const uint32_t *xx = (const uint32_t*)x, *yy = (const uint32_t*)y, *gg = (const uint32_t*)gamma, *bb = (const uint32_t*)beta;
  uint32_t *os = (uint32_t*)out_sum, *on = (uint32_t*)out_norm;
  switch (cols) {
    case 384: hipLaunchKernelGGL(k_add_layernorm<3>, g, b, 0, s, xx, yy, gg, bb, eps, rows, os, on); return true;
    case 768: hipLaunchKernelGGL(k_add_layernorm<6>, g, b, 0, s, xx, yy, gg, bb, eps, rows, os, on); return true;
    case 1024: hipLaunchKernelGGL(k_add_layernorm<8>, g, b, 0, s, xx, yy, gg, bb, eps, rows, os, on); return true;
    default: return false;
  }
}

__global__ __launch_bounds__(256) void k_upsample_bilinear_nhwc(const uint4* __restrict__ in, uint4* __restrict__ out, int ih, int iw,
                                                                int oh, int ow, int c8, float sh, float sw, long long total) {
  const long long idx = (long long)blockIdx.x * 256 + threadIdx.x;
  if (idx >= total) return;
  const int c = (int)(idx % c8);
  long long r = idx / c8;
  const int x = (int)(r % ow); r /= ow;
  const int y = (int)(r % oh);
  const long long b = r / oh;
  const float fy = sh * (float)y, fx = sw * (float)x;
  const int y0 = (int)fy, x0 = (int)fx;
  const int y1 = y0 + (y0 < ih - 1 ? 1 : 0), x1 = x0 + (x0 < iw - 1 ? 1 : 0);
  const float ly1 = fy - (float)y0, ly0 = 1.f - ly1, lx1 = fx - (float)x0, lx0 = 1.f - lx1;
  const uint4* base = in + (size_t)b * ih * iw * c8 + c;
  const uint4 p00 = base[((size_t)y0 * iw + x0) * c8], p01 = base[((size_t)y0 * iw + x1) * c8];
  const uint4 p10 = base[((size_t)y1 * iw + x0) * c8], p11 = base[((size_t)y1 * iw + x1) * c8];
  const uint32_t a00[4] = {p00.x, p00.y, p00.z, p00.w}, a01[4] = {p01.x, p01.y, p01.z, p01.w};
  const uint32_t a10[4] = {p10.x, p10.y, p10.z, p10.w}, a11[4] = {p11.x, p11.y, p11.z, p11.w};
  uint32_t o[4];
#pragma unroll
  for (int j = 0; j < 4; ++j) {
    const float lo = ly0 * (lx0 * bf2f(a00[j] & 0xffffu) + lx1 * bf2f(a01[j] & 0xffffu)) +
                     ly1 * (lx0 * bf2f(a10[j] & 0xffffu) + lx1 * bf2f(a11[j] & 0xffffu));
    const float hi = ly0 * (lx0 * bf2f(a00[j] >> 16) + lx1 * bf2f(a01[j] >> 16)) +
                     ly1 * (lx0 * bf2f(a10[j] >> 16) + lx1 * bf2f(a11[j] >> 16));
    o[j] = f2bf(lo) | (f2bf(hi) << 16);
  }
  out[idx] = make_uint4(o[0], o[1], o[2], o[3]);
}
__global__ __launch_bounds__(256) void k_upsample_bilinear_nhwc_f32(const float4* __restrict__ in, float4* __restrict__ out, int ih, int iw,
                                                                    int oh, int ow, int c4, float sh, float sw, long long total) {
  const long long idx = (long long)blockIdx.x * 256 + threadIdx.x;
  if (idx >= total) return;
  const int c = (int)(idx % c4);
  long long r = idx / c4;
  const int x = (int)(r % ow); r /= ow;
  const int y = (int)(r % oh);
  const long long b = r / oh;
  const float fy = sh * (float)y, fx = sw * (float)x;
  const int y0 = (int)fy, x0 = (int)fx;
  const int y1 = y0 + (y0 < ih - 1 ? 1 : 0), x1 = x0 + (x0 < iw - 1 ? 1 : 0);
  const float ly1 = fy - (float)y0, ly0 = 1.f - ly1, lx1 = fx - (float)x0, lx0 = 1.f - lx1;
  const float4* base = in + (size_t)b * ih * iw * c4 + c;
  const float4 p00 = base[((size_t)y0 * iw + x0) * c4], p01 = base[((size_t)y0 * iw + x1) * c4];
  const float4 p10 = base[((size_t)y1 * iw + x0) * c4], p11 = base[((size_t)y1 * iw + x1) * c4];
  float4 o;
  o.x = ly0 * (lx0 * p00.x + lx1 * p01.x) + ly1 * (lx0 * p10.x + lx1 * p11.x);
  o.y = ly0 * (lx0 * p00.y + lx1 * p01.y) + ly1 * (lx0 * p10.y + lx1 * p11.y);
  o.z = ly0 * (lx0 * p00.z + lx1 * p01.z) + ly1 * (lx0 * p10.z + lx1 * p11.z);
  o.w = ly0 * (lx0 * p00.w + lx1 * p01.w) + ly1 * (lx0 * p10.w + lx1 * p11.w);
  out[idx] = o;
}
bool vd_launch_upsample_bilinear_nhwc(hipStream_t s, int dtype, const void* in, void* out, int B, int ih, int iw, int oh, int ow, int C) {
  if (dtype == VD3D_DT_F32) {
    if (C % 4 || oh < 2 || ow < 2) return false;
    const int c4 = C / 4;
    const long long total = (long long)B * oh * ow * c4;
    const float sh = (float)(ih - 1) / (float)(oh - 1), sw = (float)(iw - 1) / (float)(ow - 1);
    hipLaunchKernelGGL(k_upsample_bilinear_nhwc_f32, dim3((unsigned)((total + 255) / 256)), dim3(256), 0, s, (const float4*)in, (float4*)out,
                       ih, iw, oh, ow, c4, sh, sw, total);
    return true;
  }
  if (dtype != VD3D_DT_BF16) return false;
  if (C % 8 || oh < 2 || ow < 2) return false;
  const int c8 = C / 8;
  const long long total = (long long)B * oh * ow * c8;
  const float sh = (float)(ih - 1) / (float)(oh - 1), sw = (float)(iw - 1) / (float)(ow - 1);
  hipLaunchKernelGGL(k_upsample_bilinear_nhwc, dim3((unsigned)((total + 255) / 256)), dim3(256), 0, s, (const uint4*)in, (uint4*)out, ih, iw,
                     oh, ow, c8, sh, sw, total);
  return true;
}

__global__ __launch_bounds__(256) void k_bias_act(const float4* __restrict__ y, const float4* __restrict__ bias, const float4* __restrict__ r1,
                                                  const float4* __restrict__ r2, int relu, int c4, long long total, float4* __restrict__ out,
                                                  float4* __restrict__ relu_out) {
  const long long idx = (long long)blockIdx.x * 256 + threadIdx.x;
  if (idx >= total) return;
  float4 v = y[idx];
  if (bias) { const float4 b = bias[(int)(idx % c4)]; v.x += b.x; v.y += b.y; v.z += b.z; v.w += b.w; }
  if (r1) { const float4 r = r1[idx]; v.x += r.x; v.y += r.y; v.z += r.z; v.w += r.w; }
  if (r2) { const float4 r = r2[idx]; v.x = r.x + v.x; v.y = r.y + v.y; v.z = r.z + v.z; v.w = r.w + v.w; }
  if (relu) { v.x = fmaxf(v.x, 0.f); v.y = fmaxf(v.y, 0.f); v.z = fmaxf(v.z, 0.f); v.w = fmaxf(v.w, 0.f); }
  out[idx] = v;
  if (relu_out) relu_out[idx] = make_float4(fmaxf(v.x, 0.f), fmaxf(v.y, 0.f), fmaxf(v.z, 0.f), fmaxf(v.w, 0.f));
}
bool vd_launch_bias_act_f32(hipStream_t s, const float* y, const float* bias, const float* r1, const float* r2, int relu, long long n_pix, int C,
                            float* out, float* relu_out) {
  if (C % 4 || n_pix < 1) return false;
  const long long total = n_pix * (C / 4);
  hipLaunchKernelGGL(k_bias_act, dim3((unsigned)((total + 255) / 256)), dim3(256), 0, s, (const float4*)y, (const float4*)bias, (const float4*)r1,
                     (const float4*)r2, relu, C / 4, total, (float4*)out, (float4*)relu_out);
  return true;
}

__global__ __launch_bounds__(256) void k_upsample_bilinear_bias_nhwc_f32(const float4* __restrict__ in, const float4* __restrict__ bias,
                                                                         float4* __restrict__ out, int ih, int iw, int oh, int ow, int c4, float sh,
                                                                         float sw, long long total) {
  const long long idx = (long long)blockIdx.x * 256 + threadIdx.x;
  if (idx >= total) return;
  const int c = (int)(idx % c4);
  long long r = idx / c4;
  const int x = (int)(r % ow); r /= ow;
  const int y = (int)(r % oh);
  const long long b = r / oh;
  const float fy = sh * (float)y, fx = sw * (float)x;
  const int y0 = (int)fy, x0 = (int)fx;
  const int y1 = y0 + (y0 < ih - 1 ? 1 : 0), x1 = x0 + (x0 < iw - 1 ? 1 : 0);
  const float ly1 = fy - (float)y0, ly0 = 1.f - ly1, lx1 = fx - (float)x0, lx0 = 1.f - lx1;
  const float4* base = in + (size_t)b * ih * iw * c4 + c;
  const float4 p00 = base[((size_t)y0 * iw + x0) * c4], p01 = base[((size_t)y0 * iw + x1) * c4];
  const float4 p10 = base[((size_t)y1 * iw + x0) * c4], p11 = base[((size_t)y1 * iw + x1) * c4];
  const float4 bb = bias[c];
  float4 o;
  o.x = (ly0 * (lx0 * p00.x + lx1 * p01.x) + ly1 * (lx0 * p10.x + lx1 * p11.x)) + bb.x;
  o.y = (ly0 * (lx0 * p00.y + lx1 * p01.y) + ly1 * (lx0 * p10.y + lx1 * p11.y)) + bb.y;
  o.z = (ly0 * (lx0 * p00.z + lx1 * p01.z) + ly1 * (lx0 * p10.z + lx1 * p11.z)) + bb.z;
  o.w = (ly0 * (lx0 * p00.w + lx1 * p01.w) + ly1 * (lx0 * p10.w + lx1 * p11.w)) + bb.w;
  out[idx] = o;
}
bool vd_launch_upsample_bilinear_bias_nhwc_f32(hipStream_t s, const float* in, const float* bias, float* out, int B, int ih, int iw, int oh, int ow, int C) {
  if (C % 4 || oh < 2 || ow < 2 || !bias) return false;
  const int c4 = C / 4;
  const long long total = (long long)B * oh * ow * c4;
  const float sh = (float)(ih - 1) / (float)(oh - 1), sw = (float)(iw - 1) / (float)(ow - 1);
  hipLaunchKernelGGL(k_upsample_bilinear_bias_nhwc_f32, dim3((unsigned)((total + 255) / 256)), dim3(256), 0, s, (const float4*)in, (const float4*)bias,
                     (float4*)out, ih, iw, oh, ow, c4, sh, sw, total);
  return true;
}

template <int LPP>
__global__ __launch_bounds__(256) void k_head_tail(const float4* __restrict__ y, const float4* __restrict__ b2, const float4* __restrict__ w3, float b3,
                                                   float scale, long long n_pix, float* __restrict__ out) {
  const long long idx = (long long)blockIdx.x * 256 + threadIdx.x;
  const long long pix = idx / LPP;
  const int l = (int)(idx % LPP);
  float acc = 0.f;
  if (pix < n_pix) {
    const float4 v = y[idx], b = b2[l], w = w3[l];
    acc = fmaxf(v.x + b.x, 0.f) * w.x;
    acc = vd_fma(fmaxf(v.y + b.y, 0.f), w.y, acc);
    acc = vd_fma(fmaxf(v.z + b.z, 0.f), w.z, acc);
    acc = vd_fma(fmaxf(v.w + b.w, 0.f), w.w, acc);
  }
#pragma unroll
  for (int off = LPP / 2; off > 0; off >>= 1) acc += __shfl_xor(acc, off, 64);
  if (l == 0 && pix < n_pix) out[pix] = fmaxf(acc + b3, 0.f) * scale;
}
bool vd_launch_head_tail_f32(hipStream_t s, const float* y, const float* b2, const float* w3, float b3, float scale, long long n_pix, int C, float* out) {
  if (n_pix < 1) return false;
  const long long total = n_pix * (C / 4);
  const dim3 g((unsigned)((total + 255) / 256)), b(256);
  const float4 *yy = (const float4*)y, *bb = (const float4*)b2, *ww = (const float4*)w3;
  switch (C) {
    case 16: hipLaunchKernelGGL(k_head_tail<4>, g, b, 0, s, yy, bb, ww, b3, scale, n_pix, out); return true;
    case 32: hipLaunchKernelGGL(k_head_tail<8>, g, b, 0, s, yy, bb, ww, b3, scale, n_pix, out); return true;
    case 64: hipLaunchKernelGGL(k_head_tail<16>, g, b, 0, s, yy, bb, ww, b3, scale, n_pix, out); return true;
    default: return false;
  }
}

__global__ __launch_bounds__(256) void k_depth_to_space_bias(const float4* __restrict__ y, const float4* __restrict__ bias, int H, int W, int s, int c4,
                                                             long long total, float4* __restrict__ out) {
  const long long idx = (long long)blockIdx.x * 256 + threadIdx.x;
  if (idx >= total) return;
  const int c = (int)(idx % c4);
  long long r = idx / c4;
  const int ow = W * s, oh = H * s;
  const int ox = (int)(r % ow); r /= ow;
  const int oy = (int)(r % oh);
  const long long b = r / oh;
  const int py = oy / s, i = oy - py * s, px = ox / s, j = ox - px * s;
  const long long p = (b * H + py) * W + px;
  float4 v = y[((p * s + i) * s + j) * c4 + c];
  if (bias) { const float4 bb = bias[c]; v.x += bb.x; v.y += bb.y; v.z += bb.z; v.w += bb.w; }
  out[idx] = v;
}
bool vd_launch_depth_to_space_bias_f32(hipStream_t s, const float* y, const float* bias, int B, int H, int W, int f, int C, float* out) {
  if (C % 4 || B < 1 || H < 1 || W < 1 || f < 1) return false;
  if ((reinterpret_cast<uintptr_t>(y) | reinterpret_cast<uintptr_t>(bias) | reinterpret_cast<uintptr_t>(out)) & 15) return false;
  const long long total = (long long)B * H * f * W * f * (C / 4);
  if ((total + 255) / 256 > 0x7fffffffLL) return false;
  hipLaunchKernelGGL(k_depth_to_space_bias, dim3((unsigned)((total + 255) / 256)), dim3(256), 0, s, (const float4*)y, (const float4*)bias, H, W, f, C / 4,
                     total, (float4*)out);
  return true;
}

__global__ __launch_bounds__(256) void k_patchify(const float* __restrict__ x, int th, int tw, int p, int gh, int gw, int kp4, long long total,
                                                  float4* __restrict__ out) {
  const long long idx = (long long)blockIdx.x * 256 + threadIdx.x;
  if (idx >= total) return;
  const int k4 = (int)(idx % kp4);
  long long r = idx / kp4;
  const int gx = (int)(r % gw); r /= gw;
  const int gy = (int)(r % gh);
  const long long b = r / gh;
  const int pp = p * p, K = 3 * pp;
  float v[4];
#pragma unroll
  for (int e = 0; e < 4; ++e) {
    const int k = k4 * 4 + e;
    v[e] = 0.f;
    if (k < K) {
      const int c = k / pp, rem = k - c * pp, ky = rem / p, kx = rem - ky * p;
      v[e] = x[((b * th + (gy * p + ky)) * tw + (gx * p + kx)) * 3 + c];
    }
  }
  out[idx] = float4{v[0], v[1], v[2], v[3]};
}
bool vd_launch_patchify_f32(hipStream_t s, const float* x, int B, int th, int tw, int p, float* out) {
  if (B < 1 || p < 1 || p > 64 || th < p || tw < p) return false;
// ... 8 lines not shown
```

visiondepth3d_amd/render_3d.py:

```python
from __future__ import annotations

import ctypes as C

import numpy as np
import torch

from . import _abi, _lib
from ._abi import DEPTH_BGR_U8, DEPTH_F32, DEPTH_GRAY_U8, DT_BF16, DT_F16, DT_F32, FORMAT_IDS, FrameScalars, LetterboxParams, LetterboxState, RenderParams, ShiftParams, State
from .geometry import aspect_ratios
from .params import reference_aten_threads, render_kwargs_to_params, shift_params_from_kwargs

torch_device = torch.device("cuda" if torch.cuda.is_available() else "cpu")


def _ptr(t: torch.Tensor):
    return C.c_void_p(t.data_ptr())


class Renderer:

    def __init__(self, device: int | torch.device | None = None, private_stream: bool = False, auto_order: bool = True):
        if not torch.cuda.is_available():
            raise RuntimeError("visiondepth3d_amd needs a ROCm GPU (MI355X); there is no CPU path")
        L = _lib.lib()
# ... 180 lines not shown
        self._enter(f, d, q_out)
        _lib.check(self._L.vd3d_shard2_p1(self._ctx, _ptr(f), _ptr(d), self._depth_fmt(d), C.byref(params), int(step_idx), int(slot),
                                          _ptr(q_out)))

    MAX_BATCH = 16

    def shard2_p1_batch(self, frames, depths, params: RenderParams, step_idx0: int, slot0: int, q_out: torch.Tensor):
        n = len(frames)
        fs = [f.to(self.device).contiguous() for f in frames]
        ds = [d.to(self.device).contiguous() for d in depths]
        fmt = self._depth_fmt(ds[0])
        if any(self._depth_fmt(d) != fmt for d in ds):
            raise AssertionError("the depth planes of one batch share one format")
        if not q_out.is_contiguous() or q_out.numel() < 2 * n:
            raise AssertionError("q_out: contiguous float32 [n, 2]")
        self._enter(q_out, *fs, *ds)
        fp = (C.c_void_p * n)(*[f.data_ptr() for f in fs])
        dp = (C.c_void_p * n)(*[d.data_ptr() for d in ds])
        _lib.check(self._L.vd3d_shard2_p1_batch(self._ctx, fp, dp, fmt, C.byref(params), int(step_idx0), int(slot0), n, _ptr(q_out)))

    def shard2_p3_batch(self, slot0: int, step_idx0: int, n: int, params: RenderParams, m_out: torch.Tensor):
        if not m_out.is_contiguous() or m_out.numel() < 4 * n:
            raise AssertionError("m_out: contiguous int64 [n, 4]")
        self._enter(m_out)
        _lib.check(self._L.vd3d_shard2_p3_batch(self._ctx, int(slot0), int(step_idx0), int(n), C.byref(params), _ptr(m_out)))

    def tdf_plane_export(self, params: RenderParams, out: torch.Tensor | None = None) -> torch.Tensor:
        if out is None:
            out = torch.empty((params.eye_h, params.eye_w), dtype=torch.float32, device=self.device)
        self._enter(out)
        _lib.check(self._L.vd3d_tdf_plane_export(self._ctx, _ptr(out), params.eye_h, params.eye_w))
        return out

    def tdf_plane_import(self, plane: torch.Tensor, params: RenderParams, valid: bool = True):
        pl = plane.to(self.device, torch.float32).contiguous()
        self._enter(pl)
        _lib.check(self._L.vd3d_tdf_plane_import(self._ctx, _ptr(pl), params.eye_h, params.eye_w, 1 if valid else 0))

    def shard2_r1(self, q_all: torch.Tensor):
        q = q_all.to(self.device, torch.float32).contiguous()
        self._enter(q)
        _lib.check(self._L.vd3d_shard2_r1(self._ctx, _ptr(q), q.numel() // 2))

    def shard2_p3(self, slot: int, step_idx: int, params: RenderParams, m_out: torch.Tensor):
        self._enter(m_out)
        _lib.check(self._L.vd3d_shard2_p3(self._ctx, int(slot), int(step_idx), C.byref(params), _ptr(m_out)))

    def shard2_r2(self, m_all: torch.Tensor, own_slots, params: RenderParams, blank=None):
        n = len(own_slots)
        arr = (C.c_int * n)(*[int(v) for v in own_slots])
        bl = (C.c_uint8 * n)(*[1 if b else 0 for b in blank]) if blank is not None else None
        m = m_all.to(self.device, torch.int64).contiguous()
        self._enter(m)
        _lib.check(self._L.vd3d_shard2_r2(self._ctx, _ptr(m), arr, bl, n, C.byref(params)))

    def set_pixel_overlap(self, on: bool):
        _lib.check(self._L.vd3d_set_pixel_overlap(self._ctx, int(on)))

    def join_pixels(self):
        _lib.check(self._L.vd3d_join_pixels(self._ctx))

    def wait_pixels(self, slot: int):
        _lib.check(self._L.vd3d_wait_pixels(self._ctx, int(slot)))

    def shard_pixels(self, slot: int, params: RenderParams, out: torch.Tensor | None = None, blank_frame: torch.Tensor | None = None):
        if out is None:
            out = torch.empty((params.out_h, params.out_w, 3), dtype=torch.uint8, device=self.device)
        if blank_frame is not None:
            f = blank_frame.to(self.device, torch.uint8).contiguous()
            self._enter(out, f)
            _lib.check(self._L.vd3d_shard_pixels_blank(self._ctx, int(slot), _ptr(f), C.byref(params), _ptr(out)))
            ps = self.pixel_stream
            if ps is not None:
                f.record_stream(ps)
                out.record_stream(ps)
            return out
        self._enter(out)
        _lib.check(self._L.vd3d_shard_pixels(self._ctx, int(slot), C.byref(params), _ptr(out)))
        if self._private and self._auto_order:
            for ps in self.pixel_streams:
                out.record_stream(ps)
        return out

    def depth_handoff(self, pred: torch.Tensor, H: int, W: int, invert: bool = False, out: torch.Tensor | None = None):
        p = pred.to(self.device, torch.float32).contiguous()
        if p.dim() == 2:
            p = p[None]
        B, ph, pw = p.shape
        if out is None:
            out = torch.empty((B, H, W), dtype=torch.uint8, device=self.device)
        self._enter(p, out)
        _lib.check(self._L.vd3d_depth_handoff(self._ctx, _ptr(p), B, ph, pw, int(H), int(W), int(bool(invert)), _ptr(out)))
        return out

    def tile_gather_cubic_u8(self, frames_bgr: torch.Tensor, origins: torch.Tensor, ch: int, cw: int, chs: int, cws: int,
                             out: torch.Tensor | None = None) -> torch.Tensor:
        f = frames_bgr if frames_bgr.dim() == 4 else frames_bgr[None]
        if f.dtype != torch.uint8 or f.dim() != 4 or f.shape[3] != 3 or f.device != self.device:
            raise AssertionError("tile_gather_cubic_u8 takes uint8 [B,H,W,3] frames on the renderer's device")
        if f.stride(3) != 1 or f.stride(2) != 3:
            f = f.contiguous()
        o = origins.to(self.device, torch.int32).contiguous()
        if o.dim() != 2 or o.shape[1] != 3:
            raise AssertionError("tile_gather_cubic_u8: origins is int32 [n,3] = (frame, y, x)")
        B, H, W, _ = f.shape
        n = int(o.shape[0])
        if out is None:
            out = torch.empty((n, int(chs), int(cws), 3), dtype=torch.uint8, device=self.device)
        self._enter(f, o, out)
        _lib.check(self._L.vd3d_tile_gather_cubic_u8(self._ctx, _ptr(f), int(f.stride(1)), int(f.stride(0)), B, H, W, _ptr(o), n,
                                                     int(ch), int(cw), int(chs), int(cws), _ptr(out)))
        return out

    def tile_blend(self, pred_pool: torch.Tensor, pred_off: torch.Tensor, tile_tab: torch.Tensor, w_pool: torch.Tensor, n_frames: int,
                   tgt_h: int, tgt_w: int, tile: int, pad: int, out: torch.Tensor | None = None) -> torch.Tensor:
        for t, dt in ((pred_pool, torch.float32), (pred_off, torch.int64), (tile_tab, torch.int32), (w_pool, torch.float32)):
            if t.dtype != dt or t.device != self.device or not t.is_contiguous():
                raise AssertionError("tile_blend: float32 pools, int64 offsets, int32 tile table, contiguous, on the renderer's device")
        if out is None:
            out = torch.empty((int(n_frames), int(tgt_h), int(tgt_w)), dtype=torch.float32, device=self.device)
        self._enter(pred_pool, pred_off, tile_tab, w_pool, out)
        _lib.check(self._L.vd3d_tile_blend_f32(self._ctx, _ptr(pred_pool), _ptr(pred_off), _ptr(tile_tab), _ptr(w_pool), int(n_frames),
                                               int(tgt_h), int(tgt_w), int(tile), int(pad), _ptr(out)))
        return out

    def depth_normalize_pclip(self, planes: torch.Tensor, invert: bool = False, pclip=(1.0, 99.0), out: torch.Tensor | None = None,
                              lo_hi: torch.Tensor | None = None) -> torch.Tensor:
        p = planes.to(self.device, torch.float32).contiguous()
        if p.dim() == 2:
            p = p[None]
        B, H, W = p.shape
        if out is None:
            out = torch.empty((B, H, W), dtype=torch.uint8, device=self.device)
        if lo_hi is not None and (lo_hi.dtype != torch.float32 or lo_hi.numel() < 2 * B or not lo_hi.is_contiguous() or lo_hi.device != self.device):
            raise AssertionError("depth_normalize_pclip: lo_hi is a contiguous float32 [B,2] tensor on the renderer's device")
        self._enter(p, out)
        _lib.check(self._L.vd3d_depth_normalize_pclip_u8(self._ctx, _ptr(p), B, H, W, float(pclip[0]), float(pclip[1]), int(bool(invert)),
                                                         _ptr(out), None if lo_hi is None else _ptr(lo_hi)))
        return out

    def _lb_frames(self, frames: torch.Tensor, what: str) -> torch.Tensor:
        f = torch.as_tensor(frames)
        f = f if f.dim() == 4 else f[None]
        if f.dtype != torch.uint8 or f.dim() != 4 or f.shape[3] != 3:
            raise AssertionError(f"{what} takes uint8 [B,H,W,3] BGR frames")
        return f.to(self.device).contiguous()

    def _lb_planes(self, planes: torch.Tensor, what: str) -> torch.Tensor:
        p = torch.as_tensor(planes)
        p = p if p.dim() == 3 else p[None]
        if p.dtype != torch.uint8 or p.dim() != 3:
            raise AssertionError(f"{what} takes uint8 [B,H,W] planes")
        return p.to(self.device).contiguous()

    def letterbox_stats(self, frames_bgr: torch.Tensor, chain: bool = False) -> dict:
        f = self._lb_frames(frames_bgr, "letterbox_stats")
        B, H, W, _ = f.shape
        dev = self.device
        o = dict(row_mean=torch.empty((B, H), dtype=torch.float32, device=dev), row_var=torch.empty((B, H), dtype=torch.float32, device=dev),
                 row_sat=torch.empty((B, H), dtype=torch.int32, device=dev), gray=torch.empty((B, H, W), dtype=torch.uint8, device=dev),
                 hist=torch.empty((B, 64), dtype=torch.int32, device=dev), mad_sum=torch.empty((B,), dtype=torch.int64, device=dev),
                 frame_mean=torch.empty((B,), dtype=torch.float32, device=dev))
        self._enter(f, *o.values())
        _lib.check(self._L.vd3d_letterbox_stats(self._ctx, _ptr(f), B, H, W, int(bool(chain)), _ptr(o["row_mean"]), _ptr(o["row_var"]), _ptr(o["row_sat"]),
                                                _ptr(o["gray"]), _ptr(o["hist"]), _ptr(o["mad_sum"]), _ptr(o["frame_mean"])))
        return o

    def canny_u8(self, gray: torch.Tensor, low: int = 30, high: int = 90, want_counts: bool = False):
        g = self._lb_planes(gray, "canny_u8")
        B, H, W = g.shape
        out = torch.empty_like(g)
        cnt = torch.empty((B, H), dtype=torch.int32, device=self.device) if want_counts else None
        self._enter(g, out, *(() if cnt is None else (cnt,)))
        _lib.check(self._L.vd3d_canny_u8(self._ctx, _ptr(g), B, H, W, int(low), int(high), _ptr(out), None if cnt is None else _ptr(cnt)))
        return (out, cnt) if want_counts else out
# ... 230 lines not shown
        if (t.dtype != torch.float16 or t.dim() != 4 or t.shape[0] != 1 or t.shape[1] != 32 or not t.is_contiguous(memory_format=torch.channels_last)):
            raise AssertionError("nhwc_f16_to_planar3 takes a [1,32,H,W] fp16 tensor in channels_last memory")
        H, W = int(t.shape[2]), int(t.shape[3])
        out = torch.empty((1, 3, H, W), dtype=torch.float32, device=self.device)
        self._enter(t, out)
        _lib.check(self._L.vd3d_nhwc_f16_to_planar3_f32(self._ctx, _ptr(t), H, W, _ptr(out)))
        return out

    def add_weighted_u8(self, a: torch.Tensor, alpha: float, b: torch.Tensor, beta: float, gamma: float = 0.0) -> torch.Tensor:
        a = a.to(self.device).contiguous()
        b = b.to(self.device).contiguous()
        if a.dtype != torch.uint8 or b.dtype != torch.uint8 or a.shape != b.shape:
            raise AssertionError("add_weighted_u8 takes two uint8 tensors of one shape")
        out = torch.empty_like(a)
        self._enter(a, b, out)
        _lib.check(self._L.vd3d_add_weighted_u8(self._ctx, _ptr(a), float(alpha), _ptr(b), float(beta), float(gamma), a.numel(), _ptr(out)))
        return out

    def heal_missing_pixels(self, warped_frame, original_frame, edge_mask=None, heal_strength=0.5) -> torch.Tensor:
        if warped_frame.dim() != 3 or warped_frame.shape[0] != 3 or warped_frame.shape != original_frame.shape:
            raise AssertionError("warped_frame and original_frame must both be [3,H,W]")
        w = warped_frame.to(self.device, torch.float32).contiguous()
        o = original_frame.to(self.device, torch.float32).contiguous()
        H, W = int(w.shape[1]), int(w.shape[2])
        e = None
        if edge_mask is not None:
            if edge_mask.numel() != H * W:
                raise AssertionError("edge_mask must be [1,H,W]")
            e = edge_mask.to(self.device, torch.float32).contiguous()
        out = torch.empty_like(w)
        self._enter(w, o, e, out)
        _lib.check(self._L.vd3d_heal_missing_pixels(self._ctx, _ptr(w), _ptr(o), _ptr(e) if e is not None else None, H, W,
                                                    float(heal_strength), _ptr(out)))
        return out

    def finish_frame(self, left, right, depth_norm, params: RenderParams, focal_depth, bar_width=0, bar_side=0):
        out = torch.empty((params.out_h, params.out_w, 3), dtype=torch.uint8, device=self.device)
        dn = depth_norm.to(self.device, torch.float32).contiguous()
        eh, ew = dn.shape[-2:]
        left, right = left.to(self.device).contiguous(), right.to(self.device).contiguous()
        self._enter(left, right, dn, out)
        _lib.check(self._L.vd3d_finish_frame(self._ctx, _ptr(left), _ptr(right), _ptr(dn), eh, ew,
                                             C.byref(params), float(focal_depth), int(bar_width), int(bar_side), _ptr(out)))
        return out

    def torch_math(self, op: str, x: torch.Tensor, param: float = 0.0) -> torch.Tensor:
        t = x.to(self.device, torch.float32).contiguous()
        o = torch.empty_like(t)
        self._enter(t, o)
        _lib.check(self._L.vd3d_torch_math(self._ctx, {"pow": 0, "sigmoid": 1, "sqrt": 2}[op], _ptr(t), float(param), _ptr(o), t.numel()))
        return o

    def torch_math_aten(self, op: str, x: torch.Tensor, param: float = 0.0, aten_threads: int = 0) -> torch.Tensor:
        t = x.to(self.device, torch.float32).contiguous()
        o = torch.empty_like(t)
        self._enter(t, o)
        _lib.check(self._L.vd3d_torch_math_aten(self._ctx, {"pow": 0, "sigmoid": 1}[op], _ptr(t), float(param), _ptr(o), t.numel(), int(aten_threads)))
        return o

    def quantiles(self, plane: torch.Tensor, qs):
        p = plane.to(self.device, torch.float32).contiguous()
        q = (C.c_float * len(qs))(*[float(np.float32(v)) for v in qs])
        o = (C.c_float * len(qs))()
        self._enter(p)
        _lib.check(self._L.vd3d_quantiles(self._ctx, _ptr(p), p.numel(), q, len(qs), o))
        return [float(v) for v in o]

    def subject_depth(self, plane: torch.Tensor) -> float:
        p = plane.to(self.device, torch.float32).contiguous()
        H, W = p.shape[-2:]
        o = C.c_float()
        self._enter(p)
        _lib.check(self._L.vd3d_subject_depth(self._ctx, _ptr(p), H, W, C.byref(o)))
        return float(o.value)

    @staticmethod
    def _dt(dtype) -> int:
        if dtype == torch.float32:
            return DT_F32
        if dtype == torch.bfloat16:
            return DT_BF16
        raise TypeError(f"depth-net glue kernels are built for float32 and bfloat16, not {dtype}")

    def depth_preprocess(self, frames_bgr: torch.Tensor, th: int, tw: int, mean, std, dtype=torch.float32) -> torch.Tensor:
        f = frames_bgr.to(self.device, torch.uint8).contiguous()
        B, H, W, _ = f.shape
        out = torch.empty((B, th, tw, 3), dtype=dtype, device=self.device)
        m = (C.c_float * 3)(*[float(v) for v in mean]); s = (C.c_float * 3)(*[float(v) for v in std])
        self._enter(f, out)
        _lib.check(self._L.vd3d_depth_preprocess(self._ctx, _ptr(f), B, H, W, int(th), int(tw), m, s, self._dt(dtype), _ptr(out)))
        return out.permute(0, 3, 1, 2)

    def add_layernorm(self, x: torch.Tensor, y, norm: torch.nn.LayerNorm):
        cols = x.shape[-1]
        rows = x.numel() // cols
        out_n = torch.empty_like(x)
        out_s = torch.empty_like(x) if y is not None else x
        self._enter(x, y, out_s, out_n)
        _lib.check(self._L.vd3d_add_layernorm(self._ctx, self._dt(x.dtype), _ptr(x), _ptr(y) if y is not None else None, _ptr(norm.weight),
                                              _ptr(norm.bias), float(norm.eps), rows, cols, _ptr(out_s) if y is not None else None, _ptr(out_n)))
        return out_s, out_n

    X3_MODES = {"bf16x3": 0, "fp16x2": 1}

    def gemm_x3_pack(self, weight: torch.Tensor, mode: str = "bf16x3") -> torch.Tensor:
        w = weight.detach().to(self.device, torch.float32).contiguous()
        N, K = w.shape
        m = self.X3_MODES[mode]
        nb = int(self._L.vd3d_gemm_x3_weight_bytes(N, K, m))
        if nb < 0:
            raise NotImplementedError(f"gemm_x3: K = {K} is not a positive multiple of 16")
        img = torch.empty(nb, dtype=torch.uint8, device=self.device)
        self._enter(w, img)
        _lib.check(self._L.vd3d_gemm_x3_pack_weights(self._ctx, _ptr(w), N, K, m, _ptr(img)))
        return img

    def linear_x3(self, x: torch.Tensor, w_image: torch.Tensor, N: int, bias: torch.Tensor | None = None, gelu: bool = False, mode: str = "bf16x3") -> torch.Tensor:
        K = x.shape[-1]
        M = x.numel() // K
        out = torch.empty(x.shape[:-1] + (int(N),), dtype=torch.float32, device=x.device)
        self._enter(x, w_image, bias, out)
        _lib.check(self._L.vd3d_gemm_x3(self._ctx, _ptr(x), M, K, _ptr(w_image), int(N), self.X3_MODES[mode], _ptr(bias) if bias is not None else None,
                                        1 if gelu else 0, _ptr(out)))
        return out

    def attention_x3(self, qkv: torch.Tensor, n_heads: int, scale: float, mode: str = "bf16x3") -> torch.Tensor:
        B, T, C3 = qkv.shape
        D = C3 // (3 * n_heads)
        if qkv.dtype != torch.float32 or not qkv.is_contiguous() or D * 3 * n_heads != C3:
            raise AssertionError("qkv must be contiguous float32 [B, T, 3 * H * D]")
        m = self.X3_MODES[mode]
        nb = int(self._L.vd3d_attention_x3_workspace_bytes(B, T, n_heads, D, m))
        if nb < 0:
            raise NotImplementedError(f"attention_x3: head size {D} not built")
        ws = getattr(self, "_attn_ws", None)
        if ws is None or ws.numel() < nb:
            ws = self._attn_ws = torch.empty(nb, dtype=torch.uint8, device=self.device)
        out = torch.empty((B, T, n_heads * D), dtype=torch.float32, device=self.device)
        self._enter(qkv, ws, out)
        _lib.check(self._L.vd3d_attention_x3(self._ctx, _ptr(qkv), B, T, n_heads, D, float(scale), m, _ptr(ws), ws.numel(), _ptr(out)))
        return out

    def attention_f32(self, qkv: torch.Tensor, n_heads: int, scale: float, form: int = 0) -> torch.Tensor:
        B, T, C3 = qkv.shape
        D = C3 // (3 * n_heads)
        if qkv.dtype != torch.float32 or not qkv.is_contiguous() or D * 3 * n_heads != C3:
            raise AssertionError("qkv must be contiguous float32 [B, T, 3 * H * D]")
        if D != 64:
            raise NotImplementedError(f"attention_f32: head size {D} not built")
        out = torch.empty((B, T, n_heads * D), dtype=torch.float32, device=self.device)
        self._enter(qkv, out)
        _lib.check(self._L.vd3d_attention_f32_form(self._ctx, _ptr(qkv), B, T, n_heads, D, float(scale), _ptr(out), int(form)))
        return out

    def conv3x3_x2_pack(self, weight: torch.Tensor):
        w = weight.detach().to(self.device, torch.float32).contiguous()
        Cout, Cin, kh, kw = w.shape
        nb = int(self._L.vd3d_conv3x3_x2_weight_bytes(Cin, Cout)) if (kh, kw) == (3, 3) else -1
        if nb < 0:
            return None
        img = torch.empty(nb, dtype=torch.uint8, device=self.device)
        self._enter(w, img)
        _lib.check(self._L.vd3d_conv3x3_x2_pack_weights(self._ctx, _ptr(w), Cin, Cout, _ptr(img)))
        return img

    def conv3x3_x2(self, x: torch.Tensor, w_image: torch.Tensor, Cout: int) -> torch.Tensor:
        B, Cin, H, W = x.shape
        if x.dtype != torch.float32 or not x.is_contiguous(memory_format=torch.channels_last):
            raise AssertionError("conv3x3_x2: float32 channels_last input")
        out = torch.empty((B, int(Cout), H, W), dtype=torch.float32, device=x.device, memory_format=torch.channels_last)
        self._enter(x, w_image, out)
        _lib.check(self._L.vd3d_conv3x3_x2(self._ctx, _ptr(x), B, H, W, Cin, _ptr(w_image), int(Cout), _ptr(out)))
        return out
# ... 347 lines not shown
```

Before: 142.2 stereo-pairs/s.

## Add LDS strip-tiled depth preprocess, separable handoff, and tiled bilinear upsample

Adds a strip-tiled antialiased downscale kernel for the depth-net preprocess. It stages source rows through LDS with register prefetch and applies separable horizontal then vertical weights. It also adds a separable form for the depth handoff upscale and rewrites the f32 NHWC bilinear upsample to share per-row coefficients across tiled rows. New form parameters (0 = auto-choose) are exposed through the C API and Python, which adds code paths whose numerics and constraints must match the general kernels.

```diff
diff --git a/include/vd3d.h b/include/vd3d.h
--- a/include/vd3d.h
+++ b/include/vd3d.h
@@ -199,6 +199,7 @@
 int vd3d_nhwc_f16_to_planar3_f32(vd3d_ctx* ctx, const void* t_nhwc32, int H, int W, float* out_planar);
 
 int vd3d_depth_handoff(vd3d_ctx* ctx, const float* pred, int B, int ph, int pw, int H, int W, int invert, uint8_t* out_gray);
+int vd3d_depth_handoff_form(vd3d_ctx* ctx, const float* pred, int B, int ph, int pw, int H, int W, int invert, uint8_t* out_gray, int form);
 
 int vd3d_tile_gather_cubic_u8(vd3d_ctx* ctx, const uint8_t* frames_bgr, long long pitch_bytes, long long frame_stride_bytes, int B, int H, int W,
                               const int32_t* origins_dev, int n, int ch, int cw, int chs, int cws, uint8_t* out_tiles);
@@ -236,6 +237,8 @@
 
 int vd3d_depth_preprocess(vd3d_ctx* ctx, const uint8_t* frames_bgr, int B, int H, int W, int th, int tw,
                           const float* mean3_host, const float* std3_host, int dtype, void* out_nhwc);
+int vd3d_depth_preprocess_form(vd3d_ctx* ctx, const uint8_t* frames_bgr, int B, int H, int W, int th, int tw,
+                               const float* mean3_host, const float* std3_host, int dtype, void* out_nhwc, int form);
 
 int vd3d_add_layernorm(vd3d_ctx* ctx, int dtype, const void* x, const void* y_or_null, const void* gamma, const void* beta,
                        float eps, int64_t rows, int cols, void* out_sum, void* out_norm);
diff --git a/visiondepth3d_amd/_lib.py b/visiondepth3d_amd/_lib.py
--- a/visiondepth3d_amd/_lib.py
+++ b/visiondepth3d_amd/_lib.py
@@ -13,9 +13,9 @@
     "vd3d_abi_version", "vd3d_last_error", "vd3d_shift_params_default", "vd3d_render_params_default",
     "vd3d_ctx_create", "vd3d_ctx_destroy", "vd3d_sync", "vd3d_ctx_stream", "vd3d_ctx_set_stream", "vd3d_ctx_pixel_stream", "vd3d_ctx_pixel_stream_k",
     "vd3d_state_reset", "vd3d_state_new_clip", "vd3d_state_export", "vd3d_state_import", "vd3d_state_planes",
-    "vd3d_last_scalars", "vd3d_pixel_shift", "vd3d_render_frame", "vd3d_render_frame_blank", "vd3d_depth_handoff", "vd3d_heal_missing_pixels", "vd3d_preview_heatmap", "vd3d_preview_arrows", "vd3d_conv3x3_c64_f16", "vd3d_conv3x3_head_f16", "vd3d_esr_tail_f32", "vd3d_conv3x3_dense_f16", "vd3d_nhwc_f16_to_planar3_f32", "vd3d_nv12_to_bgr", "vd3d_bgr_to_nv12", "vd3d_resize_cubic_u8", "vd3d_resize_area_u8", "vd3d_resize_linear_u8", "vd3d_format_3d_output", "vd3d_esr_preprocess", "vd3d_esr_postprocess", "vd3d_add_weighted_u8", "vd3d_rife_preprocess", "vd3d_rife_postprocess",
+    "vd3d_last_scalars", "vd3d_pixel_shift", "vd3d_render_frame", "vd3d_render_frame_blank", "vd3d_depth_handoff", "vd3d_depth_handoff_form", "vd3d_heal_missing_pixels", "vd3d_preview_heatmap", "vd3d_preview_arrows", "vd3d_conv3x3_c64_f16", "vd3d_conv3x3_head_f16", "vd3d_esr_tail_f32", "vd3d_conv3x3_dense_f16", "vd3d_nhwc_f16_to_planar3_f32", "vd3d_nv12_to_bgr", "vd3d_bgr_to_nv12", "vd3d_resize_cubic_u8", "vd3d_resize_area_u8", "vd3d_resize_linear_u8", "vd3d_format_3d_output", "vd3d_esr_preprocess", "vd3d_esr_postprocess", "vd3d_add_weighted_u8", "vd3d_rife_preprocess", "vd3d_rife_postprocess",
     "vd3d_shard_begin", "vd3d_shard_pixels", "vd3d_shard_pixels_blank", "vd3d_tdf_plane_export", "vd3d_tdf_plane_import", "vd3d_set_pixel_overlap", "vd3d_join_pixels", "vd3d_wait_pixels", "vd3d_finish_frame", "vd3d_quantiles",
-    "vd3d_subject_depth", "vd3d_shard2_p0", "vd3d_shard2_set_crops", "vd3d_shard2_p1", "vd3d_shard2_p1_batch", "vd3d_shard2_r1", "vd3d_shard2_p3", "vd3d_shard2_p3_batch", "vd3d_shard2_r2", "vd3d_depth_preprocess", "vd3d_tile_gather_cubic_u8", "vd3d_tile_blend_f32", "vd3d_depth_normalize_pclip_u8", "vd3d_letterbox_stats", "vd3d_canny_u8", "vd3d_canny_hysteresis_u8", "vd3d_letterbox_track", "vd3d_letterbox_state_reset", "vd3d_letterbox_state_export", "vd3d_letterbox_state_import", "vd3d_depth_letterbox_fill_u8", "vd3d_add_layernorm", "vd3d_gemm_x3_weight_bytes", "vd3d_gemm_x3_pack_weights", "vd3d_gemm_x3", "vd3d_attention_x3_workspace_bytes", "vd3d_attention_x3", "vd3d_attention_f32", "vd3d_attention_f32_form", "vd3d_conv3x3_x2_weight_bytes", "vd3d_conv3x3_x2_pack_weights", "vd3d_conv3x3_x2", "vd3d_conv3x3_x3_weight_bytes", "vd3d_conv3x3_x3_pack_weights", "vd3d_conv3x3_x3", "vd3d_conv3x3_s2_x3_weight_bytes", "vd3d_conv3x3_s2_x3_pack_weights", "vd3d_conv3x3_s2_x3", "vd3d_conv_ifn_weight_bytes", "vd3d_conv_ifn_pack_weights", "vd3d_conv_ifn", "vd3d_rife_warp_pack", "vd3d_rife_update", "vd3d_rife_blend", "vd3d_upsample_bilinear_nhwc", "vd3d_nhwc_bias_act_f32", "vd3d_upsample_bilinear_bias_nhwc_f32", "vd3d_dpt_head_tail_f32", "vd3d_dpt_head_conv_weight_bytes", "vd3d_dpt_head_conv_pack_weights", "vd3d_dpt_head_conv_f32", "vd3d_depth_to_space_bias_nhwc_f32", "vd3d_patchify_f32", "vd3d_preview_image", "vd3d_detect_black_bars", "vd3d_stream_copy", "vd3d_torch_math", "vd3d_torch_math_aten", "vd3d_debug_gaussian_kernel1d", "vd3d_debug_exp_torch", "vd3d_set_profiling", "vd3d_last_stage_ms", "vd3d_stage_calls",
+    "vd3d_subject_depth", "vd3d_shard2_p0", "vd3d_shard2_set_crops", "vd3d_shard2_p1", "vd3d_shard2_p1_batch", "vd3d_shard2_r1", "vd3d_shard2_p3", "vd3d_shard2_p3_batch", "vd3d_shard2_r2", "vd3d_depth_preprocess", "vd3d_depth_preprocess_form", "vd3d_tile_gather_cubic_u8", "vd3d_tile_blend_f32", "vd3d_depth_normalize_pclip_u8", "vd3d_letterbox_stats", "vd3d_canny_u8", "vd3d_canny_hysteresis_u8", "vd3d_letterbox_track", "vd3d_letterbox_state_reset", "vd3d_letterbox_state_export", "vd3d_letterbox_state_import", "vd3d_depth_letterbox_fill_u8", "vd3d_add_layernorm", "vd3d_gemm_x3_weight_bytes", "vd3d_gemm_x3_pack_weights", "vd3d_gemm_x3", "vd3d_attention_x3_workspace_bytes", "vd3d_attention_x3", "vd3d_attention_f32", "vd3d_attention_f32_form", "vd3d_conv3x3_x2_weight_bytes", "vd3d_conv3x3_x2_pack_weights", "vd3d_conv3x3_x2", "vd3d_conv3x3_x3_weight_bytes", "vd3d_conv3x3_x3_pack_weights", "vd3d_conv3x3_x3", "vd3d_conv3x3_s2_x3_weight_bytes", "vd3d_conv3x3_s2_x3_pack_weights", "vd3d_conv3x3_s2_x3", "vd3d_conv_ifn_weight_bytes", "vd3d_conv_ifn_pack_weights", "vd3d_conv_ifn", "vd3d_rife_warp_pack", "vd3d_rife_update", "vd3d_rife_blend", "vd3d_upsample_bilinear_nhwc", "vd3d_nhwc_bias_act_f32", "vd3d_upsample_bilinear_bias_nhwc_f32", "vd3d_dpt_head_tail_f32", "vd3d_dpt_head_conv_weight_bytes", "vd3d_dpt_head_conv_pack_weights", "vd3d_dpt_head_conv_f32", "vd3d_depth_to_space_bias_nhwc_f32", "vd3d_patchify_f32", "vd3d_preview_image", "vd3d_detect_black_bars", "vd3d_stream_copy", "vd3d_torch_math", "vd3d_torch_math_aten", "vd3d_debug_gaussian_kernel1d", "vd3d_debug_exp_torch", "vd3d_set_profiling", "vd3d_last_stage_ms", "vd3d_stage_calls",
     "vd3d_debug_planes", "vd3d_debug_tune",
 )
 
@@ -67,6 +67,7 @@
     L.vd3d_join_pixels.argtypes = [vp]
     L.vd3d_wait_pixels.argtypes = [vp, i32]
     L.vd3d_depth_handoff.argtypes = [vp, f32p, i32, i32, i32, i32, i32, i32, u8p]
+    L.vd3d_depth_handoff_form.argtypes = [vp, f32p, i32, i32, i32, i32, i32, i32, u8p, i32]
     L.vd3d_heal_missing_pixels.argtypes = [vp, f32p, f32p, f32p, i32, i32, C.c_double, f32p]
     L.vd3d_resize_cubic_u8.argtypes = [vp, u8p, i32, i32, i32, u8p, i32, i32]
     L.vd3d_nv12_to_bgr.argtypes = [vp, u8p, C.c_longlong, u8p, C.c_longlong, i32, i32, u8p]
@@ -98,6 +99,7 @@
     L.vd3d_shard2_p3.argtypes = [vp, i32, i32, vp, vp]
     L.vd3d_shard2_r2.argtypes = [vp, vp, C.POINTER(C.c_int), C.POINTER(C.c_uint8), i32, vp]
     L.vd3d_depth_preprocess.argtypes = [vp, vp, i32, i32, i32, i32, i32, C.POINTER(C.c_float), C.POINTER(C.c_float), i32, vp]
+    L.vd3d_depth_preprocess_form.argtypes = [vp, vp, i32, i32, i32, i32, i32, C.POINTER(C.c_float), C.POINTER(C.c_float), i32, vp, i32]
     L.vd3d_tile_gather_cubic_u8.argtypes = [vp, u8p, C.c_longlong, C.c_longlong, i32, i32, i32, vp, i32, i32, i32, i32, i32, u8p]
     L.vd3d_tile_blend_f32.argtypes = [vp, f32p, vp, vp, f32p, i32, i32, i32, i32, i32, f32p]
     L.vd3d_depth_normalize_pclip_u8.argtypes = [vp, f32p, i32, i32, i32, C.c_float, C.c_float, i32, u8p, f32p]
diff --git a/visiondepth3d_amd/csrc/vd3d_api.hip b/visiondepth3d_amd/csrc/vd3d_api.hip
--- a/visiondepth3d_amd/csrc/vd3d_api.hip
+++ b/visiondepth3d_amd/csrc/vd3d_api.hip
@@ -1294,14 +1294,19 @@
   return 0;
 }
 
-VD3D_EXPORT int vd3d_depth_handoff(vd3d_ctx* c, const float* pred, int B, int ph, int pw, int H, int W, int invert, uint8_t* out_gray) {
+VD3D_EXPORT int vd3d_depth_handoff_form(vd3d_ctx* c, const float* pred, int B, int ph, int pw, int H, int W, int invert, uint8_t* out_gray, int form) {
   if (!c || !pred || !out_gray || B < 1 || ph < 1 || pw < 1 || H < 1 || W < 1) return set_err(VD3D_E_INVALID, "bad argument");
+  if (form < 0 || form > 2) return set_err(VD3D_E_INVALID, "depth_handoff: form %d (0 = choose, 1 = general, 2 = separable)", form);
   HIPCHK(hipSetDevice(c->device));
   if (B > c->mm_cap) { HIPCHK(re_alloc(&c->mm, (size_t)3 * B)); c->mm_cap = B; }
   StageTimer t(c, "handoff");
-  vd_launch_depth_handoff(c->stream, pred, B, ph, pw, H, W, invert ? 1 : 0, c->mm, out_gray);
-  HIPCHK(hipGetLastError());
-  return 0;
+  if (!vd_launch_depth_handoff(c->stream, pred, B, ph, pw, H, W, invert ? 1 : 0, c->mm, out_gray, form))
+    return set_err(VD3D_E_UNSUPPORTED, "depth_handoff: the separable form is for up-scaling only (%dx%d -> %dx%d)", pw, ph, W, H);
+  HIPCHK(hipGetLastError());
+  return 0;
+}
+VD3D_EXPORT int vd3d_depth_handoff(vd3d_ctx* c, const float* pred, int B, int ph, int pw, int H, int W, int invert, uint8_t* out_gray) {
+  return vd3d_depth_handoff_form(c, pred, B, ph, pw, H, W, invert, out_gray, 0);
 }
 
 VD3D_EXPORT int vd3d_tile_gather_cubic_u8(vd3d_ctx* c, const uint8_t* frames_bgr, long long pitch_bytes, long long frame_stride_bytes, int B, int H, int W,
@@ -1443,17 +1448,23 @@
   return 0;
 }
 
-VD3D_EXPORT int vd3d_depth_preprocess(vd3d_ctx* c, const uint8_t* frames_bgr, int B, int H, int W, int th, int tw,
-                                      const float* mean3_host, const float* std3_host, int dtype, void* out_nhwc) {
+VD3D_EXPORT int vd3d_depth_preprocess_form(vd3d_ctx* c, const uint8_t* frames_bgr, int B, int H, int W, int th, int tw,
+                                           const float* mean3_host, const float* std3_host, int dtype, void* out_nhwc, int form) {
+  if (form < 0 || form > 2) return set_err(VD3D_E_INVALID, "depth_preprocess: form %d (0 = choose, 1 = general, 2 = strip)", form);
   if (dtype != VD3D_DT_BF16 && dtype != VD3D_DT_F32) return set_err(VD3D_E_INVALID, "bad dtype %d", dtype);
   if (!c || !frames_bgr || !mean3_host || !std3_host || !out_nhwc || B < 1 || H < 1 || W < 1 || th < 1 || tw < 1)
     return set_err(VD3D_E_INVALID, "bad argument");
   HIPCHK(hipSetDevice(c->device));
   StageTimer t(c, "depth_prep");
-  if (!vd_launch_depth_prep(c->stream, frames_bgr, B, H, W, th, tw, mean3_host, std3_host, dtype, out_nhwc))
-    return set_err(VD3D_E_UNSUPPORTED, "depth_preprocess: %dx%d -> %dx%d exceeds the antialias tap budget", W, H, tw, th);
-  HIPCHK(hipGetLastError());
-  return 0;
+  const int rc = vd_launch_depth_prep(c->stream, frames_bgr, B, H, W, th, tw, mean3_host, std3_host, dtype, out_nhwc, form);
+  if (rc == 1) return set_err(VD3D_E_UNSUPPORTED, "depth_preprocess: %dx%d -> %dx%d exceeds the antialias tap budget", W, H, tw, th);
+  if (rc) return set_err(VD3D_E_UNSUPPORTED, "depth_preprocess: the strip form does not hold %dx%d -> %dx%d (down-scaling within its LDS plan only)", W, H, tw, th);
+  HIPCHK(hipGetLastError());
+  return 0;
+}
+VD3D_EXPORT int vd3d_depth_preprocess(vd3d_ctx* c, const uint8_t* frames_bgr, int B, int H, int W, int th, int tw,
+                                      const float* mean3_host, const float* std3_host, int dtype, void* out_nhwc) {
+  return vd3d_depth_preprocess_form(c, frames_bgr, B, H, W, th, tw, mean3_host, std3_host, dtype, out_nhwc, 0);
 }
 
 VD3D_EXPORT int vd3d_add_layernorm(vd3d_ctx* c, int dtype, const void* x, const void* y_or_null, const void* gamma, const void* beta,
diff --git a/visiondepth3d_amd/csrc/vd3d_depthprep.hip b/visiondepth3d_amd/csrc/vd3d_depthprep.hip
--- a/visiondepth3d_amd/csrc/vd3d_depthprep.hip
+++ b/visiondepth3d_amd/csrc/vd3d_depthprep.hip
@@ -105,21 +105,135 @@
   }
 }
 
-bool vd_launch_depth_prep(hipStream_t s, const uint8_t* frames, int B, int H, int W, int th, int tw, const float mean[3],
-                          const float stdv[3], int dtype, void* out_nhwc) {
-  if (dtype != VD3D_DT_BF16 && dtype != VD3D_DT_F32) return false;
+#define DPF_SX 32
+#define DPF_BY 32
+#define DPF_HROWS 160
+#define DPF_CH 16
+#define DPF_ROWB 640
+#define DPF_RS 168
+#define DPF_NLD 11
+
+template <typename OT>
+__global__ __launch_bounds__(256) void k_depth_prep_strip(const uint8_t* __restrict__ frames, vd_prep_args a, int by, OT* __restrict__ out) {
+  __shared__ __attribute__((aligned(16))) float wx[DPF_SX * DP_KMAX];
+  __shared__ float wy[DPF_BY * DP_KMAX];
+  __shared__ int x0s[2 * DPF_SX], y0s[2 * DPF_BY];
+  __shared__ float hb[DPF_HROWS * 3 * DPF_SX];
+  __shared__ uint32_t tile[DPF_CH * DPF_RS];
+  const int tid = threadIdx.x;
+  const int ox0 = blockIdx.x * DPF_SX, oy0 = blockIdx.y * by, b = blockIdx.z;
+  if (tid < DPF_SX) {
+    int f = 0, n = 0;
+    float* w = wx + tid * DP_KMAX;
+    if (ox0 + tid < a.tw) n = dp_weights(ox0 + tid, a.W, a.scale_w, w, &f);
+    for (int j = n; j < ((n + 3) & ~3); ++j) w[j] = 0.f;
+    x0s[tid] = f; x0s[DPF_SX + tid] = n;
+  } else if (tid >= 64 && tid < 64 + by) {
+    const int t = tid - 64;
+    int f = 0, n = 0;
+    if (oy0 + t < a.th) n = dp_weights(oy0 + t, a.H, a.scale_h, wy + t * DP_KMAX, &f);
+    y0s[t] = f; y0s[DPF_BY + t] = n;
+  }
+  __syncthreads();
+  const int nx = min(DPF_SX, a.tw - ox0), ny = min(by, a.th - oy0);
+  const int c_lo = x0s[0], c_hi = x0s[nx - 1] + x0s[DPF_SX + nx - 1];
+  const int r_lo = y0s[0], r_hi = y0s[ny - 1] + y0s[DPF_BY + ny - 1];
+  const int ncol = min(c_hi - c_lo, DPF_ROWB / 3), nrow = min(r_hi - r_lo, DPF_HROWS);
+  const int rowbytes = ncol * 3;
+  const uint8_t* src = frames + (size_t)b * a.H * a.W * 3;
+  const int nch = (nrow + DPF_CH - 1) / DPF_CH;
+  const int lr = tid >> 4, ll = tid & 15;
+  uint32_t regs[DPF_NLD];
+  auto fetch = [&](int ch) {
+    const int r = ch * DPF_CH + lr;
+    const uint8_t* g = src + ((size_t)(r_lo + (r < nrow ? r : nrow - 1)) * a.W + c_lo) * 3;
+    const int ph = (int)((uintptr_t)g & 3);
+    const uint32_t* gp = reinterpret_cast<const uint32_t*>(g - ph);
+    const int ndw = (ph + rowbytes + 3) >> 2;
+#pragma unroll
+    for (int k = 0; k < DPF_NLD; ++k) regs[k] = (ll + 16 * k < ndw) ? gp[ll + 16 * k] : 0u;
+  };
+  fetch(0);
+  for (int ch = 0; ch < nch; ++ch) {
+#pragma unroll
+    for (int k = 0; k < DPF_NLD; ++k)
+      if (ll + 16 * k < DPF_RS) tile[lr * DPF_RS + ll + 16 * k] = regs[k];
+    __syncthreads();
+    if (ch + 1 < nch) fetch(ch + 1);
+#pragma unroll
+    for (int t = tid; t < DPF_CH * DPF_SX; t += 256) {
+      const int rr = t >> 5, ox = t & (DPF_SX - 1);
+      const int r = ch * DPF_CH + rr;
+      if (r >= nrow) continue;
+      float s0 = 0.f, s1 = 0.f, s2 = 0.f;
+      if (ox < nx) {
+        const int n4 = (x0s[DPF_SX + ox] + 3) >> 2;
+        const uint32_t ph = ((uint32_t)(uintptr_t)src + ((uint32_t)(r_lo + r) * (uint32_t)a.W + (uint32_t)c_lo) * 3u) & 3u;
+        const uint32_t start = ph + (uint32_t)(x0s[ox] - c_lo) * 3u;
+        const uint32_t sh = start & 3u;
+        const uint32_t* row = tile + rr * DPF_RS + (start >> 2);
+        const float4* w4 = reinterpret_cast<const float4*>(wx + ox * DP_KMAX);
+        uint32_t lo = row[0];
+        for (int g = 0; g < n4; ++g) {
+          const uint32_t d1 = row[3 * g + 1], d2 = row[3 * g + 2], d3 = row[3 * g + 3];
+          const uint32_t u0 = __builtin_amdgcn_alignbyte(d1, lo, sh), u1 = __builtin_amdgcn_alignbyte(d2, d1, sh),
+                         u2 = __builtin_amdgcn_alignbyte(d3, d2, sh);
+          lo = d3;
+          const float4 w = w4[g];
+          s0 += (float)((u0 >> 16) & 0xffu) * w.x; s1 += (float)((u0 >> 8) & 0xffu) * w.x; s2 += (float)(u0 & 0xffu) * w.x;
+          s0 += (float)((u1 >> 8) & 0xffu) * w.y;  s1 += (float)(u1 & 0xffu) * w.y;        s2 += (float)(u0 >> 24) * w.y;
+          s0 += (float)(u2 & 0xffu) * w.z;         s1 += (float)(u1 >> 24) * w.z;          s2 += (float)((u1 >> 16) & 0xffu) * w.z;
+          s0 += (float)(u2 >> 24) * w.w;           s1 += (float)((u2 >> 16) & 0xffu) * w.w; s2 += (float)((u2 >> 8) & 0xffu) * w.w;
+        }
+      }
+      float* h = hb + r * 3 * DPF_SX + ox;
+      h[0] = s0; h[DPF_SX] = s1; h[2 * DPF_SX] = s2;
+    }
+    __syncthreads();
+  }
+  for (int t = tid; t < ny * DPF_SX; t += 256) {
+    const int oy = t >> 5, ox = t & (DPF_SX - 1);
+    if (ox >= nx) continue;
+    const int rb = y0s[oy] - r_lo, n = min(y0s[DPF_BY + oy], nrow - rb);
+    const float* w = wy + oy * DP_KMAX;
+    float s[3] = {0.f, 0.f, 0.f};
+    for (int j = 0; j < n; ++j) {
+      const float* h = hb + (rb + j) * 3 * DPF_SX + ox;
+      const float wj = w[j];
+      s[0] += h[0] * wj; s[1] += h[DPF_SX] * wj; s[2] += h[2 * DPF_SX] * wj;
+    }
+    OT* o = out + (((size_t)b * a.th + (oy0 + oy)) * a.tw + (ox0 + ox)) * 3;
+#pragma unroll
+    for (int c = 0; c < 3; ++c) dp_store(o + c, ((s[c] / 255.0f) - a.mean[c]) / a.stdv[c]);
+  }
+}
+
+int vd_launch_depth_prep(hipStream_t s, const uint8_t* frames, int B, int H, int W, int th, int tw, const float mean[3],
+                         const float stdv[3], int dtype, void* out_nhwc, int form) {
+  if (dtype != VD3D_DT_BF16 && dtype != VD3D_DT_F32) return 1;
   vd_prep_args a;
   a.B = B; a.H = H; a.W = W; a.th = th; a.tw = tw;
   a.scale_h = (float)H / (float)th; a.scale_w = (float)W / (float)tw;
   const float sup_w = a.scale_w >= 1.f ? 2.f * a.scale_w : 2.f, sup_h = a.scale_h >= 1.f ? 2.f * a.scale_h : 2.f;
-  if ((int)(2.f * sup_w) + 2 > DP_KMAX || (int)(2.f * sup_h) + 2 > DP_KMAX) return false;
+  if ((int)(2.f * sup_w) + 2 > DP_KMAX || (int)(2.f * sup_h) + 2 > DP_KMAX) return 1;
   for (int c = 0; c < 3; ++c) { a.mean[c] = mean[c]; a.stdv[c] = stdv[c]; }
   a.in_cols_max = (int)(a.scale_w * DP_TX + 2.f * sup_w) + 4;
   a.in_rows_max = (int)(a.scale_h * DP_TY + 2.f * sup_h) + 4;
   size_t lds = sizeof(float) * (DP_TX + DP_TY) * DP_KMAX + sizeof(int) * 2 * (DP_TX + DP_TY) +
                sizeof(float) * (size_t)a.in_rows_max * DP_TX * 3 + (size_t)a.in_rows_max * a.in_cols_max * 3;
   lds = (lds + 15) & ~(size_t)15;
-  if (lds > 150 * 1024) return false;
+  if (lds > 150 * 1024) return 1;
+  int by = 0;
+  if (a.scale_w >= 1.f && a.scale_h >= 1.f && ((int)(a.scale_w * DPF_SX + 2.f * sup_w) + 4) * 3 <= DPF_ROWB)
+    for (by = DPF_BY; by >= 8 && (int)(a.scale_h * by + 2.f * sup_h) + 4 > DPF_HROWS; by >>= 1) {}
+  if (by < 8) by = 0;
+  if (form == 2 && !by) return 2;
+  if (form != 1 && by) {
+    dim3 g((tw + DPF_SX - 1) / DPF_SX, (th + by - 1) / by, B);
+    if (dtype == VD3D_DT_F32) hipLaunchKernelGGL(k_depth_prep_strip<float>, g, dim3(256), 0, s, frames, a, by, reinterpret_cast<float*>(out_nhwc));
+    else hipLaunchKernelGGL(k_depth_prep_strip<uint16_t>, g, dim3(256), 0, s, frames, a, by, reinterpret_cast<uint16_t*>(out_nhwc));
+    return 0;
+  }
   static bool attr[64] = {false};
   int dev = 0;
   (void)hipGetDevice(&dev);
@@ -131,5 +245,5 @@
   dim3 g((tw + DP_TX - 1) / DP_TX, (th + DP_TY - 1) / DP_TY, B);
   if (dtype == VD3D_DT_F32) hipLaunchKernelGGL(k_depth_prep<float>, g, dim3(256), lds, s, frames, a, reinterpret_cast<float*>(out_nhwc));
   else hipLaunchKernelGGL(k_depth_prep<uint16_t>, g, dim3(256), lds, s, frames, a, reinterpret_cast<uint16_t*>(out_nhwc));
-  return true;
-}
+  return 0;
+}
diff --git a/visiondepth3d_amd/csrc/vd3d_handoff.hip b/visiondepth3d_amd/csrc/vd3d_handoff.hip
--- a/visiondepth3d_amd/csrc/vd3d_handoff.hip
+++ b/visiondepth3d_amd/csrc/vd3d_handoff.hip
@@ -87,13 +87,140 @@
   }
 }
 
-void vd_launch_depth_handoff(hipStream_t s, const float* pred, int B, int ph, int pw, int H, int W, int invert, uint32_t* mm,
-                             uint8_t* out) {
+struct ho_cols { float cx[4][4]; int xs[4][4]; };
+struct ho_window { float r[4][4]; int iy; bool live; };
+
+VD_DEV void ho_cols_make(ho_cols& c, int xq, int pw, float sw) {
+#pragma unroll
+  for (int q = 0; q < 4; ++q) {
+    const float rx = vd_fma(sw, (float)(xq + q) + 0.5f, -0.5f);
+    const float fx = floorf(rx);
+    const int ix = (int)fx;
+    cubic_coeffs(rx - fx, c.cx[q]);
+#pragma unroll
+    for (int j = 0; j < 4; ++j) { int xx = ix - 1 + j; c.xs[q][j] = xx < 0 ? 0 : (xx > pw - 1 ? pw - 1 : xx); }
+  }
+}
+VD_DEV void ho_hrow(const float* __restrict__ row, const ho_cols& c, float r[4]) {
+#pragma unroll
+  for (int q = 0; q < 4; ++q) {
+    float v = 0.f;
+#pragma unroll
+    for (int j = 0; j < 4; ++j) v += row[c.xs[q][j]] * c.cx[q][j];
+    r[q] = v;
+  }
+}
+VD_DEV int ho_clamp_row(int yy, int ph) { return yy < 0 ? 0 : (yy > ph - 1 ? ph - 1 : yy); }
+VD_DEV void ho_row_values(const float* __restrict__ p, int ph, int pw, float sh, int y, const ho_cols& c, ho_window& w, float v[4]) {
+  const float ry = vd_fma(sh, (float)y + 0.5f, -0.5f);
+  const float fy = floorf(ry);
+  const int iy = __builtin_amdgcn_readfirstlane((int)fy);
+  float cy[4];
+  cubic_coeffs(ry - fy, cy);
+  if (w.live && iy == w.iy + 1) {
+#pragma unroll
+    for (int i = 0; i < 3; ++i)
+#pragma unroll
+      for (int q = 0; q < 4; ++q) w.r[i][q] = w.r[i + 1][q];
+    const int yn = ho_clamp_row(iy + 2, ph);
+    if (yn != ho_clamp_row(iy + 1, ph)) ho_hrow(p + (size_t)yn * pw, c, w.r[3]);
+  } else if (!w.live || iy != w.iy) {
+#pragma unroll
+    for (int i = 0; i < 4; ++i) {
+      const int yy = ho_clamp_row(iy - 1 + i, ph);
+      if (i > 0 && yy == ho_clamp_row(iy - 2 + i, ph)) {
+#pragma unroll
+        for (int q = 0; q < 4; ++q) w.r[i][q] = w.r[i - 1][q];
+      } else {
+        ho_hrow(p + (size_t)yy * pw, c, w.r[i]);
+      }
+    }
+  }
+  w.iy = iy; w.live = true;
+#pragma unroll
+  for (int q = 0; q < 4; ++q) {
+    float acc = 0.f;
+#pragma unroll
+    for (int i = 0; i < 4; ++i) acc += w.r[i][q] * cy[i];
+    v[q] = acc;
+  }
+}
+
+template <bool WRITE>
+__global__ __launch_bounds__(64) void k_handoff_sep(const float* __restrict__ pred, vd_handoff_args a, uint32_t* __restrict__ mm,
+                                                    uint8_t* __restrict__ out) {
+  const int b = blockIdx.z;
+  const float* p = pred + (size_t)b * a.ph * a.pw;
+  const int xq = (blockIdx.x * 64 + threadIdx.x) * 4;
+  ho_cols c;
+  ho_cols_make(c, xq, a.pw, a.sw);
+  ho_window w;
+  w.iy = 0; w.live = false;
+  float bmn = INFINITY, bmx = -INFINITY;
+  int bbad = 0;
+  float mn = 0.f, den = 1.f;
+  bool flat = false;
+  if (WRITE) {
+    const float mx = key2f(mm[3 * b + 1]);
+    mn = key2f(mm[3 * b]);
+    flat = mm[3 * b + 2] != 0u || (mx - mn) < (float)1e-6;
+    den = (mx - mn) + (float)1e-6;
+  }
+  const int y_end = min(a.H, (int)(blockIdx.y + 1) * HO_ROWS);
+  for (int y = blockIdx.y * HO_ROWS; y < y_end; ++y) {
+    float v[4];
+    ho_row_values(p, a.ph, a.pw, a.sh, y, c, w, v);
+    if (!WRITE) {
+#pragma unroll
+      for (int q = 0; q < 4; ++q)
+        if (xq + q < a.W) { bbad |= (v[q] != v[q]); bmn = v[q] < bmn ? v[q] : bmn; bmx = v[q] > bmx ? v[q] : bmx; }
+    } else {
+      if (xq >= a.W) continue;
+      uint32_t pack = 0;
+#pragma unroll
+      for (int q = 0; q < 4; ++q) {
+        uint8_t u = 0;
+        if (!flat) {
+          float n = ((v[q] - mn) / den) * 255.f;
+          n = n < 0.f ? 0.f : (n > 255.f ? 255.f : n);
+          u = (uint8_t)n;
+        }
+        if (a.invert) u = (uint8_t)(255 - u);
+        pack |= (uint32_t)u << (8 * q);
+      }
+      uint8_t* o = out + (size_t)b * a.H * a.W + (size_t)y * a.W + xq;
+      if (xq + 3 < a.W && (((size_t)b * a.H * a.W + (size_t)y * a.W + xq) & 3) == 0) *reinterpret_cast<uint32_t*>(o) = pack;
+      else for (int q = 0; q < 4 && xq + q < a.W; ++q) o[q] = (uint8_t)(pack >> (8 * q));
+    }
+  }
+  if (!WRITE) {
+    for (int off = 32; off > 0; off >>= 1) {
+      bmn = fminf(bmn, __shfl_down(bmn, off, 64));
+      bmx = fmaxf(bmx, __shfl_down(bmx, off, 64));
+      bbad |= __shfl_down(bbad, off, 64);
+    }
+    if (threadIdx.x == 0) {
+      if (bmn <= bmx) { atomicMin(&mm[3 * b], f2key(bmn)); atomicMax(&mm[3 * b + 1], f2key(bmx)); }
+      if (bbad) atomicOr(&mm[3 * b + 2], 1u);
+    }
+  }
+}
+
+bool vd_launch_depth_handoff(hipStream_t s, const float* pred, int B, int ph, int pw, int H, int W, int invert, uint32_t* mm,
+                             uint8_t* out, int form) {
   vd_handoff_args a;
   a.B = B; a.ph = ph; a.pw = pw; a.H = H; a.W = W; a.invert = invert; a.same = (ph == H && pw == W);
   a.sh = (float)ph / (float)H; a.sw = (float)pw / (float)W;
+  const bool sep_ok = !a.same && ph <= H && pw <= W;
+  if (form == 2 && !sep_ok) return false;
   hipLaunchKernelGGL(k_handoff_init, dim3((B + 63) / 64), dim3(64), 0, s, mm, B);
   dim3 g((W + 255) / 256, (H + HO_ROWS - 1) / HO_ROWS, B);
+  if (form != 1 && sep_ok) {
+    hipLaunchKernelGGL(k_handoff_sep<false>, g, dim3(64), 0, s, pred, a, mm, out);
+    hipLaunchKernelGGL(k_handoff_sep<true>, g, dim3(64), 0, s, pred, a, mm, out);
+    return true;
+  }
   hipLaunchKernelGGL(k_handoff<false>, g, dim3(256), 0, s, pred, a, mm, out);
   hipLaunchKernelGGL(k_handoff<true>, g, dim3(256), 0, s, pred, a, mm, out);
-}
+  return true;
+}
diff --git a/visiondepth3d_amd/csrc/vd3d_kernels.h b/visiondepth3d_amd/csrc/vd3d_kernels.h
--- a/visiondepth3d_amd/csrc/vd3d_kernels.h
+++ b/visiondepth3d_amd/csrc/vd3d_kernels.h
@@ -189,8 +189,8 @@
 void vd_launch_blank_eye(hipStream_t s, const uint8_t* src, int h, int w, const vd_dev_work* wk, uint8_t* dst);
 
 bool vd_launch_preview(hipStream_t s, int type, const uint8_t* L, const uint8_t* R, int h, int w, uint8_t* out);
-bool vd_launch_depth_prep(hipStream_t s, const uint8_t* frames, int B, int H, int W, int th, int tw, const float mean[3],
-                          const float stdv[3], int dtype, void* out_nhwc);
+int vd_launch_depth_prep(hipStream_t s, const uint8_t* frames, int B, int H, int W, int th, int tw, const float mean[3],
+                         const float stdv[3], int dtype, void* out_nhwc, int form);
 long long vd_gemm_x3_weight_bytes(int N, int K, int mode);
 bool vd_launch_gemm_x3_pack_w(hipStream_t s, const float* W, int N, int K, void* img, int mode);
 bool vd_launch_gemm_x3(hipStream_t s, const float* X, long long M, int K, const void* wimg, int N, const float* bias, int epilogue, float* Y, int mode);
@@ -227,8 +227,8 @@
 bool vd_launch_head_tail_f32(hipStream_t s, const float* y, const float* b2, const float* w3, float b3, float scale, long long n_pix, int C, float* out);
 bool vd_launch_depth_to_space_bias_f32(hipStream_t s, const float* y, const float* bias, int B, int H, int W, int f, int C, float* out);
 bool vd_launch_patchify_f32(hipStream_t s, const float* x, int B, int th, int tw, int p, float* out);
-void vd_launch_depth_handoff(hipStream_t s, const float* pred, int B, int ph, int pw, int H, int W, int invert, uint32_t* mm,
-                             uint8_t* out);
+bool vd_launch_depth_handoff(hipStream_t s, const float* pred, int B, int ph, int pw, int H, int W, int invert, uint32_t* mm,
+                             uint8_t* out, int form);
 
 #define VD_PCLIP_NR 6
 #define VD_PCLIP_WS_WORDS (4 * VD_PCLIP_NR * 256)
diff --git a/visiondepth3d_amd/csrc/vd3d_netops.hip b/visiondepth3d_amd/csrc/vd3d_netops.hip
--- a/visiondepth3d_amd/csrc/vd3d_netops.hip
+++ b/visiondepth3d_amd/csrc/vd3d_netops.hip
@@ -135,39 +135,86 @@
   }
   out[idx] = make_uint4(o[0], o[1], o[2], o[3]);
 }
-__global__ __launch_bounds__(256) void k_upsample_bilinear_nhwc_f32(const float4* __restrict__ in, float4* __restrict__ out, int ih, int iw,
-                                                                    int oh, int ow, int c4, float sh, float sw, long long total) {
-  const long long idx = (long long)blockIdx.x * 256 + threadIdx.x;
-  if (idx >= total) return;
-  const int c = (int)(idx % c4);
-  long long r = idx / c4;
-  const int x = (int)(r % ow); r /= ow;
-  const int y = (int)(r % oh);
-  const long long b = r / oh;
-  const float fy = sh * (float)y, fx = sw * (float)x;
-  const int y0 = (int)fy, x0 = (int)fx;
-  const int y1 = y0 + (y0 < ih - 1 ? 1 : 0), x1 = x0 + (x0 < iw - 1 ? 1 : 0);
-  const float ly1 = fy - (float)y0, ly0 = 1.f - ly1, lx1 = fx - (float)x0, lx0 = 1.f - lx1;
-  const float4* base = in + (size_t)b * ih * iw * c4 + c;
-  const float4 p00 = base[((size_t)y0 * iw + x0) * c4], p01 = base[((size_t)y0 * iw + x1) * c4];
-  const float4 p10 = base[((size_t)y1 * iw + x0) * c4], p11 = base[((size_t)y1 * iw + x1) * c4];
-  float4 o;
-  o.x = ly0 * (lx0 * p00.x + lx1 * p01.x) + ly1 * (lx0 * p10.x + lx1 * p11.x);
-  o.y = ly0 * (lx0 * p00.y + lx1 * p01.y) + ly1 * (lx0 * p10.y + lx1 * p11.y);
-  o.z = ly0 * (lx0 * p00.z + lx1 * p01.z) + ly1 * (lx0 * p10.z + lx1 * p11.z);
-  o.w = ly0 * (lx0 * p00.w + lx1 * p01.w) + ly1 * (lx0 * p10.w + lx1 * p11.w);
-  out[idx] = o;
+#define UP_YT 2
+#define UP_SPAN 256
+template <typename IT, bool BIAS>
+VD_DEV void upsample_bilinear_f32_body(const float4* __restrict__ in, const float4* __restrict__ bias, float4* __restrict__ out, int B, int ih, int iw,
+                                       int oh, int ow, int c4, int cshift, float sh, float sw) {
+  const IT e = (IT)blockIdx.x * UP_SPAN + (IT)threadIdx.x;
+  if (e >= (IT)ow * c4) return;
+  int x, c;
+  if (cshift >= 0) { x = (int)(e >> cshift); c = (int)e & (c4 - 1); }
+  else { x = (int)(e / c4); c = (int)(e - (IT)x * c4); }
+  const float fx = sw * (float)x;
+  const int x0 = (int)fx;
+  const int x1 = x0 + (x0 < iw - 1 ? 1 : 0);
+  const float lx1 = fx - (float)x0, lx0 = 1.f - lx1;
+  const IT o0 = (IT)x0 * c4 + c, o1 = (IT)x1 * c4 + c;
+  float4 bb = make_float4(0.f, 0.f, 0.f, 0.f);
+  if (BIAS) bb = bias[c];
+  for (int b = blockIdx.z; b < B; b += gridDim.z) {
+    for (int yb = blockIdx.y * UP_YT; yb < oh; yb += gridDim.y * UP_YT) {
+      float4 p00[UP_YT], p01[UP_YT], p10[UP_YT], p11[UP_YT];
+      float ly0[UP_YT], ly1[UP_YT];
+#pragma unroll
+      for (int r = 0; r < UP_YT; ++r) {
+        const int y = yb + r < oh ? yb + r : oh - 1;
+        const float fy = sh * (float)y;
+        const int y0 = __builtin_amdgcn_readfirstlane((int)fy);
+        const int y1 = y0 + (y0 < ih - 1 ? 1 : 0);
+        ly1[r] = fy - (float)y0; ly0[r] = 1.f - ly1[r];
+        const float4* r0 = in + ((size_t)b * ih + y0) * iw * c4;
+        const float4* r1 = in + ((size_t)b * ih + y1) * iw * c4;
+        p00[r] = r0[o0]; p01[r] = r0[o1]; p10[r] = r1[o0]; p11[r] = r1[o1];
+      }
+#pragma unroll
+      for (int r = 0; r < UP_YT; ++r) {
+        if (yb + r >= oh) break;
+        float4 o;
+        o.x = ly0[r] * (lx0 * p00[r].x + lx1 * p01[r].x) + ly1[r] * (lx0 * p10[r].x + lx1 * p11[r].x);
+        o.y = ly0[r] * (lx0 * p00[r].y + lx1 * p01[r].y) + ly1[r] * (lx0 * p10[r].y + lx1 * p11[r].y);
+        o.z = ly0[r] * (lx0 * p00[r].z + lx1 * p01[r].z) + ly1[r] * (lx0 * p10[r].z + lx1 * p11[r].z);
+        o.w = ly0[r] * (lx0 * p00[r].w + lx1 * p01[r].w) + ly1[r] * (lx0 * p10[r].w + lx1 * p11[r].w);
+        if (BIAS) { o.x = o.x + bb.x; o.y = o.y + bb.y; o.z = o.z + bb.z; o.w = o.w + bb.w; }
+        (out + ((size_t)b * oh + (yb + r)) * ow * c4)[e] = o;
+      }
+    }
+  }
+}
+template <typename IT>
+__global__ __launch_bounds__(UP_SPAN) void k_upsample_bilinear_nhwc_f32(const float4* __restrict__ in, float4* __restrict__ out, int B, int ih, int iw,
+                                                                        int oh, int ow, int c4, int cshift, float sh, float sw) {
+  upsample_bilinear_f32_body<IT, false>(in, nullptr, out, B, ih, iw, oh, ow, c4, cshift, sh, sw);
+}
+template <typename IT>
+__global__ __launch_bounds__(UP_SPAN) void k_upsample_bilinear_bias_nhwc_f32(const float4* __restrict__ in, const float4* __restrict__ bias,
+                                                                             float4* __restrict__ out, int B, int ih, int iw, int oh, int ow, int c4,
+                                                                             int cshift, float sh, float sw) {
+  upsample_bilinear_f32_body<IT, true>(in, bias, out, B, ih, iw, oh, ow, c4, cshift, sh, sw);
+}
+static bool launch_upsample_bilinear_f32(hipStream_t s, const float* in, const float* bias, float* out, int B, int ih, int iw, int oh, int ow, int C) {
+  if (C % 4 || oh < 2 || ow < 2) return false;
+  const int c4 = C / 4;
+  const int cshift = (c4 & (c4 - 1)) ? -1 : __builtin_ctz((unsigned)c4);
+  const float sh = (float)(ih - 1) / (float)(oh - 1), sw = (float)(iw - 1) / (float)(ow - 1);
+  const long long rowq = (long long)ow * c4, inq = (long long)iw * c4;
+  const long long gx = (rowq + UP_SPAN - 1) / UP_SPAN, gy = ((long long)oh + UP_YT - 1) / UP_YT;
+  if (gx > 0x7fffffffll) return false;
+  const dim3 g((unsigned)gx, (unsigned)(gy < 65535 ? gy : 65535), (unsigned)(B < 65535 ? B : 65535));
+  const bool wide = rowq >= (1ll << 31) - UP_SPAN || inq >= (1ll << 31);
+  const float4 *i4 = (const float4*)in, *b4 = (const float4*)bias;
+  float4* o4 = (float4*)out;
+  if (bias) {
+    if (wide) hipLaunchKernelGGL(k_upsample_bilinear_bias_nhwc_f32<long long>, g, dim3(UP_SPAN), 0, s, i4, b4, o4, B, ih, iw, oh, ow, c4, cshift, sh, sw);
+    else hipLaunchKernelGGL(k_upsample_bilinear_bias_nhwc_f32<int>, g, dim3(UP_SPAN), 0, s, i4, b4, o4, B, ih, iw, oh, ow, c4, cshift, sh, sw);
+  } else {
+    if (wide) hipLaunchKernelGGL(k_upsample_bilinear_nhwc_f32<long long>, g, dim3(UP_SPAN), 0, s, i4, o4, B, ih, iw, oh, ow, c4, cshift, sh, sw);
+    else hipLaunchKernelGGL(k_upsample_bilinear_nhwc_f32<int>, g, dim3(UP_SPAN), 0, s, i4, o4, B, ih, iw, oh, ow, c4, cshift, sh, sw);
+  }
+  return true;
 }
 bool vd_launch_upsample_bilinear_nhwc(hipStream_t s, int dtype, const void* in, void* out, int B, int ih, int iw, int oh, int ow, int C) {
-  if (dtype == VD3D_DT_F32) {
-    if (C % 4 || oh < 2 || ow < 2) return false;
-    const int c4 = C / 4;
-    const long long total = (long long)B * oh * ow * c4;
-    const float sh = (float)(ih - 1) / (float)(oh - 1), sw = (float)(iw - 1) / (float)(ow - 1);
-    hipLaunchKernelGGL(k_upsample_bilinear_nhwc_f32, dim3((unsigned)((total + 255) / 256)), dim3(256), 0, s, (const float4*)in, (float4*)out,
-                       ih, iw, oh, ow, c4, sh, sw, total);
-    return true;
-  }
+  if (dtype == VD3D_DT_F32) return launch_upsample_bilinear_f32(s, (const float*)in, nullptr, (float*)out, B, ih, iw, oh, ow, C);
   if (dtype != VD3D_DT_BF16) return false;
   if (C % 8 || oh < 2 || ow < 2) return false;
   const int c8 = C / 8;
@@ -200,39 +247,9 @@
   return true;
 }
 
-__global__ __launch_bounds__(256) void k_upsample_bilinear_bias_nhwc_f32(const float4* __restrict__ in, const float4* __restrict__ bias,
-                                                                         float4* __restrict__ out, int ih, int iw, int oh, int ow, int c4, float sh,
-                                                                         float sw, long long total) {
-  const long long idx = (long long)blockIdx.x * 256 + threadIdx.x;
-  if (idx >= total) return;
-  const int c = (int)(idx % c4);
-  long long r = idx / c4;
-  const int x = (int)(r % ow); r /= ow;
-  const int y = (int)(r % oh);
-  const long long b = r / oh;
-  const float fy = sh * (float)y, fx = sw * (float)x;
-  const int y0 = (int)fy, x0 = (int)fx;
-  const int y1 = y0 + (y0 < ih - 1 ? 1 : 0), x1 = x0 + (x0 < iw - 1 ? 1 : 0);
-  const float ly1 = fy - (float)y0, ly0 = 1.f - ly1, lx1 = fx - (float)x0, lx0 = 1.f - lx1;
-  const float4* base = in + (size_t)b * ih * iw * c4 + c;
-  const float4 p00 = base[((size_t)y0 * iw + x0) * c4], p01 = base[((size_t)y0 * iw + x1) * c4];
-  const float4 p10 = base[((size_t)y1 * iw + x0) * c4], p11 = base[((size_t)y1 * iw + x1) * c4];
-  const float4 bb = bias[c];
-  float4 o;
-  o.x = (ly0 * (lx0 * p00.x + lx1 * p01.x) + ly1 * (lx0 * p10.x + lx1 * p11.x)) + bb.x;
-  o.y = (ly0 * (lx0 * p00.y + lx1 * p01.y) + ly1 * (lx0 * p10.y + lx1 * p11.y)) + bb.y;
-  o.z = (ly0 * (lx0 * p00.z + lx1 * p01.z) + ly1 * (lx0 * p10.z + lx1 * p11.z)) + bb.z;
-  o.w = (ly0 * (lx0 * p00.w + lx1 * p01.w) + ly1 * (lx0 * p10.w + lx1 * p11.w)) + bb.w;
-  out[idx] = o;
-}
 bool vd_launch_upsample_bilinear_bias_nhwc_f32(hipStream_t s, const float* in, const float* bias, float* out, int B, int ih, int iw, int oh, int ow, int C) {
-  if (C % 4 || oh < 2 || ow < 2 || !bias) return false;
-  const int c4 = C / 4;
-  const long long total = (long long)B * oh * ow * c4;
-  const float sh = (float)(ih - 1) / (float)(oh - 1), sw = (float)(iw - 1) / (float)(ow - 1);
-  hipLaunchKernelGGL(k_upsample_bilinear_bias_nhwc_f32, dim3((unsigned)((total + 255) / 256)), dim3(256), 0, s, (const float4*)in, (const float4*)bias,
-                     (float4*)out, ih, iw, oh, ow, c4, sh, sw, total);
-  return true;
+  if (!bias) return false;
+  return launch_upsample_bilinear_f32(s, in, bias, out, B, ih, iw, oh, ow, C);
 }
 
 template <int LPP>
diff --git a/visiondepth3d_amd/render_3d.py b/visiondepth3d_amd/render_3d.py
--- a/visiondepth3d_amd/render_3d.py
+++ b/visiondepth3d_amd/render_3d.py
@@ -286,7 +286,7 @@
                 out.record_stream(ps)
         return out
 
-    def depth_handoff(self, pred: torch.Tensor, H: int, W: int, invert: bool = False, out: torch.Tensor | None = None):
+    def depth_handoff(self, pred: torch.Tensor, H: int, W: int, invert: bool = False, out: torch.Tensor | None = None, form: int = 0):
         p = pred.to(self.device, torch.float32).contiguous()
         if p.dim() == 2:
             p = p[None]
@@ -294,7 +294,7 @@
         if out is None:
             out = torch.empty((B, H, W), dtype=torch.uint8, device=self.device)
         self._enter(p, out)
-        _lib.check(self._L.vd3d_depth_handoff(self._ctx, _ptr(p), B, ph, pw, int(H), int(W), int(bool(invert)), _ptr(out)))
+        _lib.check(self._L.vd3d_depth_handoff_form(self._ctx, _ptr(p), B, ph, pw, int(H), int(W), int(bool(invert)), _ptr(out), int(form)))
         return out
 
     def tile_gather_cubic_u8(self, frames_bgr: torch.Tensor, origins: torch.Tensor, ch: int, cw: int, chs: int, cws: int,
@@ -691,13 +691,13 @@
             return DT_BF16
         raise TypeError(f"depth-net glue kernels are built for float32 and bfloat16, not {dtype}")
 
-    def depth_preprocess(self, frames_bgr: torch.Tensor, th: int, tw: int, mean, std, dtype=torch.float32) -> torch.Tensor:
+    def depth_preprocess(self, frames_bgr: torch.Tensor, th: int, tw: int, mean, std, dtype=torch.float32, form: int = 0) -> torch.Tensor:
         f = frames_bgr.to(self.device, torch.uint8).contiguous()
         B, H, W, _ = f.shape
         out = torch.empty((B, th, tw, 3), dtype=dtype, device=self.device)
         m = (C.c_float * 3)(*[float(v) for v in mean]); s = (C.c_float * 3)(*[float(v) for v in std])
         self._enter(f, out)
-        _lib.check(self._L.vd3d_depth_preprocess(self._ctx, _ptr(f), B, H, W, int(th), int(tw), m, s, self._dt(dtype), _ptr(out)))
+        _lib.check(self._L.vd3d_depth_preprocess_form(self._ctx, _ptr(f), B, H, W, int(th), int(tw), m, s, self._dt(dtype), _ptr(out), int(form)))
         return out.permute(0, 3, 1, 2)
 
     def add_layernorm(self, x: torch.Tensor, y, norm: torch.nn.LayerNorm):
```

Result: faster. 144.2 stereo-pairs/s, median of 6 (+1.4%).
